# skygazer42/realtime-video-analytics-32streams

Measured on AMD Instinct MI355X. Metric: aggregate detected FPS across streams + p99 per-frame latency, 32x1080p30, higher is better.
Workload: dtype f16

## Files before the change

### include/rva.h

```cpp
#ifndef RVA_H
#define RVA_H

#include <stdint.h>

#ifdef __cplusplus
extern "C" {
#endif

#define RVA_ABI_VERSION 1

enum rva_status {
    RVA_OK = 0,
    RVA_ERR_ARG = 1,
    RVA_ERR_HIP = 2,
    RVA_ERR_CAPACITY = 3,
    RVA_ERR_UNAVAILABLE = 4
};

enum rva_dtype { RVA_F16 = 0, RVA_F32 = 1, RVA_F64 = 2  };

typedef struct rva_ctx rva_ctx;
typedef struct rva_tracker rva_tracker;
typedef void *rva_stream_t;

// ... 104 lines not shown
#define RVA_SNAPSHOT_SLOTS 8
int rva_tracker_snapshot_async(rva_tracker *trk, int slot, rva_stream_t stream);
int rva_tracker_snapshot_fetch(rva_tracker *trk, int slot, int wait, int64_t *ids, int32_t *cls, int32_t *age,
                               int32_t *hits, double *conf, double *boxes, int32_t *last_det,
                               int32_t *counts);

int rva_tracker_snapshot_status(rva_tracker *trk, int slot, int32_t *emitted, int32_t *processed, int32_t *flags);

int rva_tracker_state(rva_tracker *trk, int64_t *next_id, int *flags, rva_stream_t stream);
int rva_tracker_set_next_id(rva_tracker *trk, int64_t next_id, rva_stream_t stream);

int rva_conv_cout_pad(int Cout);
int rva_conv_num_variants(void);
const char *rva_conv_variant_name(int variant);
int rva_conv2d_nhwc_f16(rva_ctx *ctx, const void *in, int ldi, const void *weights, const float *bias,
                        void *out, int ldo, const void *residual, int ldr, int batch, int H, int W, int Cin,
                        int Cout, int ksize, int stride, int act, rva_stream_t stream);
int rva_conv2d_nhwc_f16_v(rva_ctx *ctx, const void *in, int ldi, const void *weights, const float *bias,
                          void *out, int ldo, const void *residual, int ldr, int batch, int H, int W, int Cin,
                          int Cout, int ksize, int stride, int act, int variant, rva_stream_t stream);
int rva_conv2d_nhwc_f16_rows(rva_ctx *ctx, const void *in, int ldi, const void *weights, const float *bias,
                             void *out, int ldo, const void *residual, int ldr, int batch, int H, int W, int Cin,
                             int Cout, int ksize, int stride, int act, int variant, int y0, int y1, rva_stream_t stream);
int rva_conv_rows_through(int k, int stride, int H_in, int lo, int hi, int32_t *out_lo, int32_t *out_hi);
int rva_conv1x1_upcat_f16(rva_ctx *ctx, const void *low, int ld_low, int c_low, const void *skip, int ld_skip,
                          int c_skip, const void *weights, const float *bias, void *out, int ldo, int batch,
                          int H, int W, int Cout, int act, int variant, rva_stream_t stream);
int rva_conv1x1_head_f16(rva_ctx *ctx, const void *in, int ldi, const void *weights, const float *bias, int batch,
                         int H, int W, int Cin, int Cout, int mode, void *out, int nc, int anchors_total,
                         int anchor_offset, float stride_px, int variant, rva_stream_t stream);
int rva_conv1x1_head_box32_f16(rva_ctx *ctx, const void *in, int ldi, const void *weights, const float *bias, int batch,
                               int H, int W, int Cin, void *out, float *boxes32, int nc, int anchors_total, int anchor_offset,
                               float stride_px, int variant, rva_stream_t stream);
int rva_stem_conv_f16(rva_ctx *ctx, const void *in_planar, const void *weights, const float *bias,
                      void *out, int ldo, int batch, int H, int W, int Cout, rva_stream_t stream);

int rva_c2f_pair32_f16(rva_ctx *ctx, const void *in, int ldi, const void *w1, const float *b1, const void *w2, const float *b2, void *out,
                       int ldo, int batch, int H, int W, rva_stream_t stream);

int rva_stem2_f16(rva_ctx *ctx, const void *in_planar, const void *w1, const float *b1, const void *w2, const float *b2,
                  void *out, int ldo, int batch, int H, int W, rva_stream_t stream);
int rva_stem2_f16_rows(rva_ctx *ctx, const void *in_planar, const void *w1, const float *b1, const void *w2, const float *b2,
                       void *out, int ldo, int batch, int H, int W, int y0, int y1, rva_stream_t stream);

int rva_sppf_pool3_nhwc_f16(rva_ctx *ctx, const void *in, int ldi, void *out1, void *out2, void *out3, int ldo,
                            int batch, int H, int W, int C, rva_stream_t stream);
int rva_maxpool5_nhwc_f16(rva_ctx *ctx, const void *in, int ldi, void *out, int ldo, int batch, int H,
                          int W, int C, rva_stream_t stream);
int rva_upsample2x_nhwc_f16(rva_ctx *ctx, const void *in, int ldi, void *out, int ldo, int batch, int H,
                            int W, int C, rva_stream_t stream);
int rva_yolo_head_f16(rva_ctx *ctx, const void *box_logits, int ldb, const void *cls_logits, int ldc,
                      void *out, int batch, int h, int w, int nc, int anchors_total, int anchor_offset,
                      float stride, rva_stream_t stream);
int rva_yolo_head3_f16(rva_ctx *ctx, const void *const *box_logits, const int32_t *ldb, const void *const *cls_logits,
                       const int32_t *ldc, void *out, int batch, const int32_t *h, const int32_t *w, int nc,
                       int anchors_total, const float *strides, rva_stream_t stream);
int rva_yolo_head_box32_f16(rva_ctx *ctx, const void *box_logits, int ldb, const void *cls_logits, int ldc, void *out,
                            float *boxes32, int batch, int h, int w, int nc, int anchors_total, int anchor_offset, float stride,
                            rva_stream_t stream);
int rva_yolo_head3_box32_f16(rva_ctx *ctx, const void *const *box_logits, const int32_t *ldb, const void *const *cls_logits,
                             const int32_t *ldc, void *out, float *boxes32, int batch, const int32_t *h, const int32_t *w, int nc,
                             int anchors_total, const float *strides, rva_stream_t stream);

int rva_conv_f32_num_variants(void);
int rva_conv2d_nhwc_f32_v(rva_ctx *ctx, const void *in, int ldi, const void *weights, const float *bias,
                          void *out, int ldo, const void *residual, int ldr, int batch, int H, int W, int Cin,
                          int Cout, int ksize, int stride, int act, int variant, rva_stream_t stream);
int rva_stem_conv_f32(rva_ctx *ctx, const void *in_planar, const void *weights, const float *bias,
                      void *out, int ldo, int batch, int H, int W, int Cout, rva_stream_t stream);
int rva_maxpool5_nhwc_f32(rva_ctx *ctx, const void *in, int ldi, void *out, int ldo, int batch, int H,
                          int W, int C, rva_stream_t stream);
int rva_upsample2x_nhwc_f32(rva_ctx *ctx, const void *in, int ldi, void *out, int ldo, int batch, int H,
                            int W, int C, rva_stream_t stream);
int rva_yolo_head_f32(rva_ctx *ctx, const void *box_logits, int ldb, const void *cls_logits, int ldc,
                      void *out, int batch, int h, int w, int nc, int anchors_total, int anchor_offset,
                      float stride, rva_stream_t stream);

#define RVA_PLAN_NO_STEM2 1
#define RVA_PLAN_NO_CIN_PAD 2
#define RVA_PLAN_NO_PAIR32 4
#define RVA_PLAN_F32 8
#define RVA_PLAN_BOX_F32 16
typedef struct rva_yolov8_plan rva_yolov8_plan;
typedef struct rva_yolov8_desc {
    int32_t batch, height, width;
    int32_t widths[5];
    int32_t depth_backbone[4];
    int32_t depth_head;
    int32_t nc, reg_max;
    int32_t n_convs;
    int32_t flags;
} rva_yolov8_desc;
typedef struct rva_conv_weights {
    const float *weight;
    const float *bias;
    int32_t cout, cin, k, stride;
} rva_conv_weights;
int rva_yolov8_plan_create(rva_ctx *ctx, const rva_yolov8_desc *desc, const rva_conv_weights *convs, rva_yolov8_plan **out);
void rva_yolov8_plan_destroy(rva_yolov8_plan *plan);
int rva_yolov8_plan_info(const rva_yolov8_plan *plan, int32_t *anchors, int32_t *out_rows, int32_t *n_steps, int32_t *n_tunable,
                         int32_t *quiet_step);
int rva_yolov8_plan_output_layout(const rva_yolov8_plan *plan, int64_t *total_bytes, int64_t *boxes_offset);
int rva_yolov8_plan_run(rva_yolov8_plan *plan, const void *input, void *output, rva_stream_t stream);
int rva_yolov8_plan_run_lanes(rva_yolov8_plan *plan, const void *input, void *output, rva_stream_t stream, rva_stream_t side1,
                              rva_stream_t side2);
int rva_yolov8_plan_run_range(rva_yolov8_plan *plan, const void *input, void *output, int first, int last, rva_stream_t stream);
int rva_yolov8_plan_tunable_desc(const rva_yolov8_plan *plan, int index, char *buf, int len);
int rva_yolov8_plan_launch_tunable(rva_yolov8_plan *plan, int index, int variant, void *output, rva_stream_t stream);
int rva_yolov8_plan_set_variant(rva_yolov8_plan *plan, int index, int variant);
int rva_yolov8_plan_get_variant(const rva_yolov8_plan *plan, int index);
int rva_yolov8_plan_set_static_rows(rva_yolov8_plan *plan, int top, int bottom);
int rva_yolov8_plan_run_n(rva_yolov8_plan *plan, const void *input, void *output, int n, rva_stream_t stream);
int rva_yolov8_plan_run_lanes_n(rva_yolov8_plan *plan, const void *input, void *output, int n, rva_stream_t stream, rva_stream_t side1,
                                rva_stream_t side2);
int rva_yolov8_plan_run_range_n(rva_yolov8_plan *plan, const void *input, void *output, int n, int first, int last, rva_stream_t stream);
// ... 179 lines not shown
```

### realtime_video_analytics_32streams_amd/_native.py

```python
from __future__ import annotations

import ctypes as C
import os
import shutil
import subprocess
from pathlib import Path
from typing import Optional

PKG = Path(__file__).resolve().parent
ROOT = PKG.parent
CSRC = PKG / "csrc"
LIB_PATH = Path(os.environ["RVA_LIB_PATH"]) if os.environ.get("RVA_LIB_PATH") else PKG / "librva.so"
SOURCES = ["rva_ctx.hip", "rva_preprocess.hip", "rva_postprocess.hip", "rva_tracker.hip", "rva_conv.hip", "rva_conv_f32.hip", "rva_plan.hip", "rva_clip.hip",
           "rva_clip3d.hip", "rva_clip3d_f16.hip", "rva_clip_f16.hip", "rva_resnet.hip", "rva_resnet_f16.hip", "rva_gates.hip", "rva_decode.hip", "rva_preview.hip", "rva_jpeg.hip"]
HIPCC_FLAGS = ["--offload-arch=gfx950", "-O3", "-fPIC", "-shared", "-std=c++17", "-ffp-contract=off",
               "-Wall", "-Wno-unused-function"]

RVA_OK, RVA_ERR_ARG, RVA_ERR_HIP, RVA_ERR_CAPACITY, RVA_ERR_UNAVAILABLE = range(5)
RVA_F16, RVA_F32, RVA_F64 = 0, 1, 2
NORM_IMAGENET_F32, NORM_VIDEO_F32, NORM_IMAGENET_F64 = 0, 1, 2
LAYOUT_NCHW, LAYOUT_CNHW = 0, 1
RVA_MAX_BATCH = 64
RVA_CODEC_H264, RVA_CODEC_HEVC = 0, 1

# ... 26 lines not shown
class CnnLstmWeights(C.Structure):
    NAMES = ("conv1_w", "conv1_b", "conv2_w", "conv2_b", "w_ih1", "b1", "w_hh1", "w_ih2", "w_hh2", "b2", "head_w", "head_b")
    _fields_ = [(n, C.POINTER(C.c_float)) for n in NAMES]


class Cnn3dDesc(C.Structure):
    _fields_ = [("height", C.c_int32), ("width", C.c_int32), ("frames", C.c_int32), ("classes", C.c_int32), ("max_clips", C.c_int32)]


class Cnn3dWeights(C.Structure):
    NAMES = ("conv1_w", "conv1_b", "conv2_w", "conv2_b", "conv3_w", "conv3_b", "head_w", "head_b")
    _fields_ = [(n, C.POINTER(C.c_float)) for n in NAMES]


class ResNetDesc(C.Structure):
    _fields_ = [("height", C.c_int32), ("width", C.c_int32), ("classes", C.c_int32), ("top_k", C.c_int32), ("max_frames", C.c_int32)]


class ResNetWeights(C.Structure):
    NAMES = ("stem_w", "stem_b") + tuple(f"c{i}_{x}" for i in range(19) for x in "wb") + ("head_w", "head_b")
    _fields_ = [(n, C.POINTER(C.c_float)) for n in NAMES]


class PreviewItem(C.Structure):
    _fields_ = [("y", C.c_void_p), ("uv", C.c_void_p), ("out_bgr", C.c_void_p)] + [
        (n, C.c_int32) for n in ("pitch", "src_w", "src_h", "ratio", "dst_w", "dst_h", "rect_first", "n_rects", "glyph_first", "n_glyphs")]


RVA_PLAN_NO_STEM2 = 1
RVA_PLAN_NO_CIN_PAD = 2
RVA_PLAN_NO_PAIR32 = 4
RVA_PLAN_F32 = 8
RVA_PLAN_BOX_F32 = 16


def _stale() -> bool:
    if not LIB_PATH.exists():
        return True
    t = LIB_PATH.stat().st_mtime
    deps = [CSRC / s for s in SOURCES] + [CSRC / "rva_internal.h", CSRC / "rva_mfma_f32.h", CSRC / "rva_mfma_f16.h", ROOT / "include" / "rva.h"]
    return any(d.exists() and d.stat().st_mtime > t for d in deps)


def build(force: bool = False, verbose: bool = False) -> Path:
    if not force and not _stale():
        return LIB_PATH
    hipcc = shutil.which("hipcc") or "/opt/rocm/bin/hipcc"
    if not Path(hipcc).exists():
        if LIB_PATH.exists():
            return LIB_PATH
        raise RuntimeError("hipcc not found and librva.so is not built")
    cmd = [hipcc, *HIPCC_FLAGS, f"-I{ROOT / 'include'}", "-o", str(LIB_PATH), *[str(CSRC / s) for s in SOURCES], "-ldl"]
    if verbose:
        print(" ".join(cmd))
    subprocess.check_call(cmd, cwd=str(CSRC))
    return LIB_PATH


_LIB: Optional[C.CDLL] = None
_P = C.c_void_p


def lib() -> C.CDLL:
    global _LIB
    if _LIB is not None:
        return _LIB
# ... 45 lines not shown
        "rva_tracker_set_gates": (C.c_int, [_P, i32p, i32p, i32p, i32p, C.c_int]),
        "rva_tracker_snapshot_status": (C.c_int, [_P, C.c_int, _P, _P, C.POINTER(C.c_int32)]),
        "rva_tracker_new_counts": (_P, [_P]),
        "rva_tracker_assign_ids": (C.c_int, [_P, _P, C.c_int, i32p, _P]),
        "rva_tracker_read": (C.c_int, [_P, C.c_int, C.c_int, _P, _P, _P, _P, _P, _P, _P, i32p, _P]),
        "rva_tracker_read_all": (C.c_int, [_P, _P, _P, _P, _P, _P, _P, _P, _P, _P]),
        "rva_tracker_snapshot_async": (C.c_int, [_P, C.c_int, _P]),
        "rva_tracker_snapshot_fetch": (C.c_int, [_P, C.c_int, C.c_int, _P, _P, _P, _P, _P, _P, _P, _P]),
        "rva_tracker_state": (C.c_int, [_P, i64p, C.POINTER(C.c_int), _P]),
        "rva_tracker_set_next_id": (C.c_int, [_P, C.c_int64, _P]),
        "rva_preview_nv12": (C.c_int, [_P, _P, _P, C.c_int, C.c_int, C.c_int, C.c_int, _P, C.c_int, C.c_int, _P, _P, C.c_int, _P, C.c_int,
                                       C.c_int, _P]),
        "rva_decode_available": (C.c_int, [C.c_char_p, C.c_int]),
        "rva_decoder_create": (C.c_int, [_P, C.c_int, C.c_int, C.POINTER(_P)]),
        "rva_decoder_destroy": (None, [_P]),
        "rva_decoder_feed": (C.c_int, [_P, C.c_char_p, C.c_int, C.c_int64, C.c_int]),
        "rva_decoder_next_frame": (C.c_int, [_P, C.POINTER(_P), C.POINTER(_P), i32p, i32p, i32p, i64p, i32p]),
        "rva_decoder_release": (C.c_int, [_P, C.c_int]),
        "rva_motion_nv12_batch": (C.c_int, [_P, pp, pp, i32p, pp, pp, C.c_int, C.c_int, C.c_int, _P, _P]),
        "rva_motion_nv12_masked_batch": (C.c_int, [_P, pp, pp, i32p, pp, pp, pp, C.c_int, C.c_int, C.c_int, _P, _P]),
        "rva_motion_bgr_batch": (C.c_int, [_P, pp, i32p, pp, pp, C.c_int, C.c_int, C.c_int, _P, _P]),
        "rva_preprocess_nv12_masked_batch": (C.c_int, [_P, pp, pp, i32p, pp, C.c_int, C.c_int, C.c_int, _P, C.c_int, C.c_int,
                                                       C.c_int, C.POINTER(Letterbox), _P]),
        "rva_resize_nv12_to_bgr_batch": (C.c_int, [_P, pp, pp, i32p, pp, C.c_int, C.c_int, C.c_int, _P, C.c_int, C.c_int, _P]),
        "rva_tracker_set_box_scale": (C.c_int, [_P, f64p]),
        "rva_conv_cout_pad": (C.c_int, [C.c_int]),
        "rva_conv_num_variants": (C.c_int, []),
        "rva_conv_variant_name": (C.c_char_p, [C.c_int]),
        "rva_conv2d_nhwc_f16": (C.c_int, [_P, _P, C.c_int, _P, _P, _P, C.c_int, _P, C.c_int] + [C.c_int] * 8 + [_P]),
        "rva_conv2d_nhwc_f16_v": (C.c_int, [_P, _P, C.c_int, _P, _P, _P, C.c_int, _P, C.c_int] + [C.c_int] * 9 + [_P]),
        "rva_conv2d_nhwc_f16_rows": (C.c_int, [_P, _P, C.c_int, _P, _P, _P, C.c_int, _P, C.c_int] + [C.c_int] * 11 + [_P]),
        "rva_conv_rows_through": (C.c_int, [C.c_int] * 5 + [i32p, i32p]),
        "rva_stem2_f16_rows": (C.c_int, [_P, _P, _P, _P, _P, _P, _P, C.c_int, C.c_int, C.c_int, C.c_int, C.c_int, C.c_int, _P]),
        "rva_stem_conv_f16": (C.c_int, [_P, _P, _P, _P, _P, C.c_int, C.c_int, C.c_int, C.c_int, C.c_int, _P]),
        "rva_stem2_f16": (C.c_int, [_P, _P, _P, _P, _P, _P, _P, C.c_int, C.c_int, C.c_int, C.c_int, _P]),
        "rva_c2f_pair32_f16": (C.c_int, [_P, _P, C.c_int, _P, _P, _P, _P, _P, C.c_int, C.c_int, C.c_int, C.c_int, _P]),
        "rva_conv1x1_head_f16": (C.c_int, [_P, _P, C.c_int, _P, _P, C.c_int, C.c_int, C.c_int, C.c_int, C.c_int, C.c_int, _P, C.c_int,
                                           C.c_int, C.c_int, C.c_float, C.c_int, _P]),
        "rva_conv1x1_head_box32_f16": (C.c_int, [_P, _P, C.c_int, _P, _P, C.c_int, C.c_int, C.c_int, C.c_int, _P, _P, C.c_int,
                                                 C.c_int, C.c_int, C.c_float, C.c_int, _P]),
        "rva_yolo_head_box32_f16": (C.c_int, [_P, _P, C.c_int, _P, C.c_int, _P, _P, C.c_int, C.c_int, C.c_int, C.c_int, C.c_int,
                                              C.c_int, C.c_float, _P]),
        "rva_yolo_head3_box32_f16": (C.c_int, [_P, pp, i32p, pp, i32p, _P, _P, C.c_int, i32p, i32p, C.c_int, C.c_int,
                                               C.POINTER(C.c_float), _P]),
        "rva_conv1x1_upcat_f16": (C.c_int, [_P, _P, C.c_int, C.c_int, _P, C.c_int, C.c_int, _P, _P, _P, C.c_int, C.c_int, C.c_int,
                                            C.c_int, C.c_int, C.c_int, C.c_int, _P]),
        "rva_yolo_head3_f16": (C.c_int, [_P, pp, i32p, pp, i32p, _P, C.c_int, i32p, i32p, C.c_int, C.c_int, C.POINTER(C.c_float), _P]),
        "rva_sppf_pool3_nhwc_f16": (C.c_int, [_P, _P, C.c_int, _P, _P, _P, C.c_int, C.c_int, C.c_int, C.c_int, C.c_int, _P]),
        "rva_maxpool5_nhwc_f16": (C.c_int, [_P, _P, C.c_int, _P, C.c_int, C.c_int, C.c_int, C.c_int, C.c_int, _P]),
        "rva_upsample2x_nhwc_f16": (C.c_int, [_P, _P, C.c_int, _P, C.c_int, C.c_int, C.c_int, C.c_int, C.c_int, _P]),
        "rva_yolo_head_f16": (C.c_int, [_P, _P, C.c_int, _P, C.c_int, _P, C.c_int, C.c_int, C.c_int, C.c_int, C.c_int,
                                        C.c_int, C.c_float, _P]),
        "rva_conv_f32_num_variants": (C.c_int, []),
        "rva_conv2d_nhwc_f32_v": (C.c_int, [_P, _P, C.c_int, _P, _P, _P, C.c_int, _P, C.c_int] + [C.c_int] * 9 + [_P]),
        "rva_stem_conv_f32": (C.c_int, [_P, _P, _P, _P, _P, C.c_int, C.c_int, C.c_int, C.c_int, C.c_int, _P]),
        "rva_maxpool5_nhwc_f32": (C.c_int, [_P, _P, C.c_int, _P, C.c_int, C.c_int, C.c_int, C.c_int, C.c_int, _P]),
        "rva_upsample2x_nhwc_f32": (C.c_int, [_P, _P, C.c_int, _P, C.c_int, C.c_int, C.c_int, C.c_int, C.c_int, _P]),
        "rva_yolo_head_f32": (C.c_int, [_P, _P, C.c_int, _P, C.c_int, _P, C.c_int, C.c_int, C.c_int, C.c_int, C.c_int,
                                        C.c_int, C.c_float, _P]),
        "rva_yolov8_plan_create": (C.c_int, [_P, C.POINTER(YoloV8Desc), C.POINTER(ConvWeights), C.POINTER(_P)]),
        "rva_yolov8_plan_destroy": (None, [_P]),
        "rva_yolov8_plan_info": (C.c_int, [_P, i32p, i32p, i32p, i32p, i32p]),
        "rva_yolov8_plan_output_layout": (C.c_int, [_P, i64p, i64p]),
        "rva_yolov8_plan_run": (C.c_int, [_P, _P, _P, _P]),
        "rva_yolov8_plan_run_lanes": (C.c_int, [_P, _P, _P, _P, _P, _P]),
        "rva_yolov8_plan_run_range": (C.c_int, [_P, _P, _P, C.c_int, C.c_int, _P]),
# ... 59 lines not shown
        raise RuntimeError("librva.so ABI version mismatch; rebuild it")
    _LIB = L
    return L


EXPORTS = [
    "rva_abi_version", "rva_create", "rva_destroy", "rva_last_error", "rva_reserve", "rva_letterbox_meta",
    "rva_preprocess_nv12_batch", "rva_preprocess_nv12_content_batch", "rva_preprocess_bgr_batch", "rva_preprocess_clip_nv12_batch",
    "rva_preprocess_clip_bgr_batch", "rva_profile_next_preprocess", "rva_preprocess_frames_nv12_batch", "rva_preprocess_frames_bgr_batch", "rva_postprocess_batch", "rva_post_status", "rva_post_filter_stats", "rva_tracker_create",
    "rva_tracker_destroy", "rva_tracker_update_f32", "rva_tracker_update_f64", "rva_tracker_update_gated_f32",
    "rva_tracker_set_gates", "rva_tracker_snapshot_status", "rva_tracker_new_counts",
    "rva_tracker_assign_ids", "rva_tracker_read", "rva_tracker_read_all", "rva_tracker_snapshot_async",
    "rva_tracker_snapshot_fetch", "rva_tracker_state",
    "rva_tracker_set_next_id", "rva_preview_nv12", "rva_decode_available", "rva_decoder_create", "rva_decoder_destroy", "rva_decoder_feed",
    "rva_decoder_next_frame", "rva_decoder_release", "rva_motion_nv12_batch", "rva_motion_nv12_masked_batch", "rva_motion_bgr_batch",
    "rva_preprocess_nv12_masked_batch", "rva_resize_nv12_to_bgr_batch", "rva_tracker_set_box_scale", "rva_conv_cout_pad", "rva_conv_num_variants", "rva_conv_variant_name", "rva_conv2d_nhwc_f16", "rva_conv2d_nhwc_f16_v", "rva_stem_conv_f16", "rva_stem2_f16", "rva_c2f_pair32_f16",
    "rva_conv1x1_head_f16", "rva_conv1x1_upcat_f16", "rva_sppf_pool3_nhwc_f16", "rva_maxpool5_nhwc_f16", "rva_upsample2x_nhwc_f16", "rva_yolo_head_f16", "rva_yolo_head3_f16",
    "rva_conv_f32_num_variants", "rva_conv2d_nhwc_f32_v", "rva_stem_conv_f32", "rva_maxpool5_nhwc_f32", "rva_upsample2x_nhwc_f32",
    "rva_yolo_head_f32",
    "rva_postprocess_boxes_batch", "rva_conv1x1_head_box32_f16", "rva_yolo_head_box32_f16", "rva_yolo_head3_box32_f16",
    "rva_yolov8_plan_output_layout",
    "rva_yolov8_plan_create", "rva_yolov8_plan_destroy", "rva_yolov8_plan_info", "rva_yolov8_plan_run", "rva_yolov8_plan_run_lanes",
    "rva_yolov8_plan_run_range", "rva_yolov8_plan_tunable_desc", "rva_yolov8_plan_launch_tunable", "rva_yolov8_plan_set_variant",
    "rva_yolov8_plan_get_variant", "rva_yolov8_plan_set_static_rows", "rva_yolov8_plan_step_rows", "rva_yolov8_plan_run_n",
    "rva_yolov8_plan_run_lanes_n", "rva_yolov8_plan_run_range_n", "rva_yolov8_plan_primed_images", "rva_conv2d_nhwc_f16_rows",
    "rva_stem2_f16_rows", "rva_conv_rows_through", "rva_cnnlstm_plan_create", "rva_cnnlstm_plan_destroy", "rva_cnnlstm_plan_info", "rva_cnnlstm_plan_run",
    "rva_cnnlstm_plan_run_post", "rva_cnnlstm_plan_stage", "rva_cnnlstm_f16_plan_create", "rva_cnnlstm_f16_plan_destroy", "rva_cnnlstm_f16_plan_info",
    "rva_cnnlstm_f16_plan_run", "rva_cnnlstm_f16_plan_run_post", "rva_cnnlstm_f16_plan_stage", "rva_cnn3d_plan_create", "rva_cnn3d_plan_destroy", "rva_cnn3d_plan_info", "rva_cnn3d_plan_run",
    "rva_cnn3d_plan_run_post", "rva_cnn3d_plan_stage", "rva_cnn3d_f16_plan_create", "rva_cnn3d_f16_plan_destroy", "rva_cnn3d_f16_plan_info",
    "rva_cnn3d_f16_plan_run", "rva_cnn3d_f16_plan_run_post", "rva_cnn3d_f16_plan_stage", "rva_resnet_plan_create", "rva_resnet_plan_destroy", "rva_resnet_plan_info",
    "rva_resnet_plan_run", "rva_resnet_plan_run_post", "rva_resnet_plan_stage", "rva_resnet_f16_plan_create", "rva_resnet_f16_plan_destroy",
    "rva_resnet_f16_plan_info", "rva_resnet_f16_plan_run", "rva_resnet_f16_plan_run_post", "rva_resnet_f16_plan_stage", "rva_jpeg_max_bytes", "rva_jpeg_encode_bgr", "rva_jpeg_status",
    "rva_jpeg_batch_create", "rva_jpeg_batch_destroy", "rva_jpeg_batch_encode", "rva_preview_nv12_batch",
]


class Context:

    def __init__(self, device: int = 0):
        L = lib()
        h = _P()
        rc = L.rva_create(device, C.byref(h))
        if rc != RVA_OK or not h:
            raise RuntimeError(
                f"rva_create(device={device}) failed with status {rc}: no usable HIP device. "
                "The MI355X hot path has no CPU fallback.")
        self.handle = h
        self.device = device

    def check(self, rc: int, what: str = "") -> None:
        if rc != RVA_OK:
            msg = lib().rva_last_error(self.handle)
            raise RuntimeError(f"{what or 'librva'} failed (status {rc}): {msg.decode() if msg else ''}")

    def close(self) -> None:
        if getattr(self, "handle", None):
            lib().rva_destroy(self.handle)
            self.handle = None

    def __del__(self):
        try:
            self.close()
        except Exception:
            pass


# ... 17 lines not shown
```

### realtime_video_analytics_32streams_amd/csrc/rva_conv.hip

```cpp
#include <hip/hip_fp16.h>

#include <cstdlib>

#include "rva_internal.h"

namespace {

typedef _Float16 h8 __attribute__((ext_vector_type(8)));
typedef float f4 __attribute__((ext_vector_type(4)));
typedef unsigned int u4 __attribute__((ext_vector_type(4)));

struct ConvArgs {
    const __half *in; int ldi;
    const __half *w;
    const float *bias;
    __half *out; int ldo;
    union {
        const __half *res;
        float *hbox;
    };
    int ldr;
    int CoutPad;
    __half *hout; int hmode, hnc, hA, ha0, hW, hHW; float hstride;
    const __half *in2; int ldi2, c_split;
// ... 996 lines not shown
        for (int t = 0; t < 16; ++t) mx = fmaxf(mx, v[t]);
        float se = 0.f, sw = 0.f;
#pragma unroll
        for (int t = 0; t < 16; ++t) { const float e = __expf(v[t] - mx); se += e; sw += e * (float)t; }
        d[s] = sw / se;
    }
    const float ax = (float)(i % a.w) + 0.5f, ay = (float)(i / a.w) + 0.5f;
    const float x1 = ax - d[0], y1 = ay - d[1], x2 = ax + d[2], y2 = ay + d[3];
    __half *o = a.out + (size_t)b * (4 + a.nc) * a.A + a.a0 + i;
    o[0] = __float2half_rn((x1 + x2) * 0.5f * a.stride);
    o[(size_t)a.A] = __float2half_rn((y1 + y2) * 0.5f * a.stride);
    o[(size_t)2 * a.A] = __float2half_rn((x2 - x1) * a.stride);
    o[(size_t)3 * a.A] = __float2half_rn((y2 - y1) * a.stride);
    if constexpr (BOX32) {
        float *o32 = box32 + (size_t)b * 4 * a.A + a.a0 + i;
        o32[0] = (x1 + x2) * 0.5f * a.stride;
        o32[(size_t)a.A] = (y1 + y2) * 0.5f * a.stride;
        o32[(size_t)2 * a.A] = (x2 - x1) * a.stride;
        o32[(size_t)3 * a.A] = (y2 - y1) * a.stride;
    }
    const __half *cp = a.cls + pix * a.ldc;
    for (int c = 0; c < a.nc; c += 8) {
        const uint4 q = *reinterpret_cast<const uint4 *>(cp + c);
        const __half2 *hq = reinterpret_cast<const __half2 *>(&q);
#pragma unroll
        for (int t = 0; t < 4; ++t) {
            const float2 f = __half22float2(hq[t]);
            o[(size_t)(4 + c + 2 * t) * a.A] = __float2half_rn(__builtin_amdgcn_rcpf(1.0f + __expf(-f.x)));
            o[(size_t)(5 + c + 2 * t) * a.A] = __float2half_rn(__builtin_amdgcn_rcpf(1.0f + __expf(-f.y)));
        }
    }
}

struct BigArgs {
    const __half *in; int ldi;
    const __half *w; const float *bias;
    __half *out; int ldo;
    const __half *res; int ldr;
    int H, W, Cin, Cout, CoutPad, act, n_tiles, M, m_tiles;
};

typedef __attribute__((address_space(3))) void *lds_vptr;
typedef const __attribute__((address_space(1))) void *glb_vptr;

template <int N> __device__ __forceinline__ void wait_vm() { asm volatile("s_waitcnt vmcnt(%0)" ::"n"(N) : "memory"); }

__device__ __forceinline__ void lds_dma16(unsigned voff, const void *sbase, unsigned m0v)
{
    const unsigned long long b = (unsigned long long)(size_t)sbase;
    const unsigned lo = __builtin_amdgcn_readfirstlane((unsigned)b), hi = __builtin_amdgcn_readfirstlane((unsigned)(b >> 32));
    const unsigned long long sb = ((unsigned long long)hi << 32) | lo;
    const unsigned m0s = __builtin_amdgcn_readfirstlane(m0v);
    asm volatile("s_mov_b32 m0, %2\n\ts_nop 0\n\tglobal_load_lds_dwordx4 %0, %1" ::"v"(voff), "s"(sb), "s"(m0s) : "memory");
}
__device__ __forceinline__ void lds_dma16_masked(unsigned voff, const void *sbase, unsigned m0v, unsigned long long mask)
{
    const unsigned long long b = (unsigned long long)(size_t)sbase;
    const unsigned lo = __builtin_amdgcn_readfirstlane((unsigned)b), hi = __builtin_amdgcn_readfirstlane((unsigned)(b >> 32));
    const unsigned long long sb = ((unsigned long long)hi << 32) | lo;
    const unsigned m0s = __builtin_amdgcn_readfirstlane(m0v);
    const unsigned mlo = __builtin_amdgcn_readfirstlane((unsigned)mask), mhi = __builtin_amdgcn_readfirstlane((unsigned)(mask >> 32));
    const unsigned long long ms = ((unsigned long long)mhi << 32) | mlo;
    asm volatile("s_mov_b32 m0, %2\n\ts_mov_b64 exec, %3\n\tglobal_load_lds_dwordx4 %0, %1\n\ts_mov_b64 exec, -1" ::"v"(voff), "s"(sb), "s"(m0s), "s"(ms) : "memory");
}
__device__ __forceinline__ unsigned lds_addr(const void *p) { return (unsigned)(size_t)(lds_vptr)p; }
__device__ __forceinline__ void wait_vm_n(int n)
{
    switch (n) {
    case 0: wait_vm<0>(); break;
    case 1: wait_vm<1>(); break;
    case 2: wait_vm<2>(); break;
    case 3: wait_vm<3>(); break;
    case 4: wait_vm<4>(); break;
    case 5: wait_vm<5>(); break;
    case 6: wait_vm<6>(); break;
    case 7: wait_vm<7>(); break;
    case 8: wait_vm<8>(); break;
    case 9: wait_vm<9>(); break;
    case 10: wait_vm<10>(); break;
    case 11: wait_vm<11>(); break;
    case 12: wait_vm<12>(); break;
    default: wait_vm<12>(); break;
    }
}

template <int BM, int BN, int WGM, int WGN, int NSLOT>
__global__ void __launch_bounds__(512) __attribute__((amdgpu_waves_per_eu(NSLOT == 2 ? 4 : 2))) k_conv3_big(BigArgs a)
{
    static_assert(WGM * WGN == 8, "eight waves");
    static_assert(NSLOT == 2 || NSLOT == 3, "ring depth");
    constexpr int TM = BM / WGM, TN = BN / WGN, FM = TM / 16, FN = TN / 16;
    constexpr int APIECES = (BM + 2 + 15) / 16;
    constexpr int WPIECES = 3 * BN / 16;
    constexpr int PIECES = APIECES + WPIECES;
    constexpr int SLOTH = PIECES * 512;
    constexpr int NP = (PIECES + 7) / 8;
    extern __shared__ __attribute__((aligned(16))) unsigned char smem[];
    __half *ring = (__half *)smem;

    const int tid = threadIdx.x, lane = tid & 63;
    const int wv = __builtin_amdgcn_readfirstlane(tid >> 6);
    const int wm = wv % WGM, wn = wv / WGM;
    const int n_tile = (blockIdx.x >> 3) % a.n_tiles, m_tile = ((blockIdx.x >> 3) / a.n_tiles) * 8 + (blockIdx.x & 7);
    if (m_tile >= a.m_tiles) return;
    const int P0 = m_tile * BM, n0 = n_tile * BN;
    const int HW = a.H * a.W;
    const int cpt = a.Cin >> 5;
    const int nsteps = 3 * cpt;
    const int wrow = 9 * a.Cin;

    const int lrow = lane >> 2, lp = lane & 3;
    const int my_pieces = (PIECES - wv + 7) / 8;
    unsigned poff0[NP], poff1[NP], poff2[NP];
#pragma unroll
    for (int k = 0; k < NP; ++k) {
        const int idx = wv + 8 * k;
        if (idx < APIECES) {
            const int r = idx * 16 + lrow;
            const unsigned c = (unsigned)(((lp - 2 * (r >> 2)) & 3) * 16);
            const int q1 = P0 - 1 + r;
// ... 129 lines not shown
                    if (!((vm[j] >> (vsh + dx)) & 1)) bf[0][j] = hz;
                }
#pragma unroll
                for (int i = 0; i < FN; ++i) {
                    const h8 a1 = *reinterpret_cast<const h8 *>(wb + swz32(dx * BN + wn * TN + i * 16 + (lane & 15), ch));
#pragma unroll
                    for (int j = 0; j < FM; ++j) acc[i][j] = __builtin_amdgcn_mfma_f32_16x16x32_f16(a1, bf[0][j], acc[i][j], 0, 0, 0);
                }
            }
        }
        if (NSLOT == 3 && more && !early) BIG_ISSUE();
        STAMP(5);
    }
    __syncthreads();

    constexpr int SROW = BN + 8;
    __half *stage = (__half *)smem;
#pragma unroll
    for (int i = 0; i < FN; ++i) {
        const int co = wn * TN + 16 * i + (lane >> 4) * 4;
        const float4 bv = bvs[i];
#pragma unroll
        for (int j = 0; j < FM; ++j) {
            float v0 = acc[i][j][0] + bv.x, v1 = acc[i][j][1] + bv.y, v2 = acc[i][j][2] + bv.z, v3 = acc[i][j][3] + bv.w;
            if (a.act) { v0 = silu_f(v0); v1 = silu_f(v1); v2 = silu_f(v2); v3 = silu_f(v3); }
            const int px = wm * TM + 16 * j + (lane & 15);
            __half2 lo = __floats2half2_rn(v0, v1), hi = __floats2half2_rn(v2, v3);
            uint2 pk;
            pk.x = *reinterpret_cast<uint32_t *>(&lo);
            pk.y = *reinterpret_cast<uint32_t *>(&hi);
            *reinterpret_cast<uint2 *>(stage + (size_t)px * SROW + co) = pk;
        }
    }
    __syncthreads();
    constexpr int CPR = BN / 8;
#pragma unroll 4
    for (int q = tid; q < BM * CPR; q += 512) {
        const int row = q / CPR, pc = q - row * CPR;
        const int co = n0 + pc * 8;
        const int m = P0 + row;
        if (m < a.M && co < a.Cout) {
            uint4 v = *reinterpret_cast<const uint4 *>(stage + (size_t)row * SROW + pc * 8);
            if (a.res) {
                const uint4 r = *reinterpret_cast<const uint4 *>(a.res + (size_t)m * a.ldr + co);
                __half2 *vh = reinterpret_cast<__half2 *>(&v);
                const __half2 *rh = reinterpret_cast<const __half2 *>(&r);
#pragma unroll
                for (int u = 0; u < 4; ++u) {
                    const float2 x = __half22float2(vh[u]), y = __half22float2(rh[u]);
                    vh[u] = __floats2half2_rn(x.x + y.x, x.y + y.y);
                }
            }
            *reinterpret_cast<uint4 *>(a.out + (size_t)m * a.ldo + co) = v;
        }
    }
    STAMP(6);
}

#undef BIG_ISSUE
#undef BIG_ISSUE_ADVANCE
#undef BIG_ISSUE_PIECE

template <int BM, int BN, int WGM, int WGN, int NSLOT>
hipError_t launch_big(BigArgs &a, hipStream_t s)
{
    constexpr size_t ring = (size_t)NSLOT * ((BM + 2 + 15) / 16 + 3 * BN / 16) * 1024;
    constexpr size_t st = (size_t)BM * (BN + 8) * 2;
    constexpr size_t smem = ring > st ? ring : st;
    static_assert(smem <= 160 * 1024, "LDS budget");
    if (a.Cin % 32 || a.CoutPad % 4 || a.M >= (1 << 24)) return hipErrorInvalidValue;
    if ((size_t)a.M * a.ldi * 2 >= (1ull << 32) || (size_t)a.CoutPad * 9 * a.Cin * 2 >= (1ull << 32)) return hipErrorInvalidValue;
    if (hipError_t e = rva_func_smem((const void *)k_conv3_big<BM, BN, WGM, WGN, NSLOT>, smem); e != hipSuccess) return e;
    a.n_tiles = rva_ceil_div(a.Cout, BN);
    a.m_tiles = rva_ceil_div(a.M, BM);
    k_conv3_big<BM, BN, WGM, WGN, NSLOT><<<rva_ceil_div(a.m_tiles, 8) * 8 * a.n_tiles, 512, smem, s>>>(a);
    return hipGetLastError();
}

struct RunArgs {
    const __half *in; int ldi;
    const __half *w; const float *bias;
    __half *out; int ldo;
    const __half *res; int ldr;
    int H, W, Cin, Cout, CoutPad, act, n_tiles, M, m_tiles, apieces, map_off;
};

template <int BM, int BN, int WGM, int WGN, bool NOSEL = false, bool PADO = false>
__global__ void __launch_bounds__(512) __attribute__((amdgpu_waves_per_eu(BN <= 64 && BM <= 320 ? 4 : 2))) k_conv3_run(RunArgs a)
{
    static_assert(WGM * WGN == 8, "eight waves");
    constexpr int TM = BM / WGM, TN = BN / WGN, FM = TM / 16, FN = TN / 16;
    constexpr int WPIECES = 3 * BN / 16;
    constexpr int NPW = (WPIECES + 7) / 8;
    constexpr int MAXA = 5;
    extern __shared__ __attribute__((aligned(16))) unsigned char smem[];
    const int tid = threadIdx.x, lane = tid & 63;
    const int wv = __builtin_amdgcn_readfirstlane(tid >> 6);
    const int wm = wv % WGM, wn = wv / WGM;
    const int n_tile = (blockIdx.x >> 3) % a.n_tiles, m_tile = ((blockIdx.x >> 3) / a.n_tiles) * 8 + (blockIdx.x & 7);
    if (m_tile >= a.m_tiles) return;
    const int P0 = m_tile * BM, n0 = n_tile * BN;
    const int HW = a.H * a.W;
    const int cpt = a.Cin >> 5;
    const int nsteps = 3 * cpt;
    const int wrow = 9 * a.Cin;
    const int apieces = a.apieces;
    __half *act0 = (__half *)smem;
    __half *wt0 = act0 + (size_t)2 * apieces * 512;
    const unsigned lds_act = lds_addr(act0), lds_w = lds_addr(wt0);

    const int lrow = lane >> 2, lp = lane & 3;
    unsigned aoff[MAXA], woff[NPW];
    const int Wp = PADO ? a.W + 1 : a.W, HWp = (a.H + 1) * Wp;
    const float inv_wp = 1.0f / (float)Wp, inv_hwp = 1.0f / (float)HWp;
    unsigned long long amask[PADO ? MAXA : 1];
    auto pixel_of = [&](int pos) {
        if (pos < 0) return -1;
        const int b = div_s(pos, HWp, inv_hwp), rem = pos - b * HWp, yy = div_s(rem, Wp, inv_wp), xx = rem - yy * Wp;
        const int m = (b * a.H + yy) * a.W + xx;
        return (yy < a.H && xx < a.W && m < a.M) ? m : -1;
    };
// ... 123 lines not shown
        RUN_LOAD(0, 0);
        RUN_LOAD(1, 1);
        RUN_MFMA(0, 0);
        if (!early) RUN_ISSUE();
        RUN_LOAD(0, 2);
        RUN_MFMA(1, 1);
        RUN_MFMA(0, 2);
#undef RUN_LOAD
#undef RUN_MFMA
#undef RUN_ISSUE
        cc = ncc; dy = ndy;
        STAMP(5);
    }
    __syncthreads();

    constexpr int SROW = BN + 8;
    __half *stage = (__half *)smem;
#pragma unroll
    for (int i = 0; i < FN; ++i) {
        const int co = wn * TN + 16 * i + (lane >> 4) * 4;
        const float4 bv = bvs[i];
#pragma unroll
        for (int j = 0; j < FM; ++j) {
            float v0 = acc[i][j][0] + bv.x, v1 = acc[i][j][1] + bv.y, v2 = acc[i][j][2] + bv.z, v3 = acc[i][j][3] + bv.w;
            if (a.act) { v0 = silu_f(v0); v1 = silu_f(v1); v2 = silu_f(v2); v3 = silu_f(v3); }
            const int px = wm * TM + 16 * j + (lane & 15);
            __half2 lo = __floats2half2_rn(v0, v1), hi = __floats2half2_rn(v2, v3);
            uint2 pk;
            pk.x = *reinterpret_cast<uint32_t *>(&lo);
            pk.y = *reinterpret_cast<uint32_t *>(&hi);
            *reinterpret_cast<uint2 *>(stage + (size_t)px * SROW + co) = pk;
        }
    }
    __syncthreads();
    constexpr int CPR = BN / 8;
#pragma unroll 4
    for (int q = tid; q < BM * CPR; q += 512) {
        const int row = q / CPR, pc = q - row * CPR;
        const int co = n0 + pc * 8;
        const int m = PADO ? rowmap[row] : P0 + row;
        if ((PADO ? m >= 0 : m < a.M) && co < a.Cout) {
            uint4 v = *reinterpret_cast<const uint4 *>(stage + (size_t)row * SROW + pc * 8);
            if (a.res) {
                const uint4 r = *reinterpret_cast<const uint4 *>(a.res + (size_t)m * a.ldr + co);
                __half2 *vh = reinterpret_cast<__half2 *>(&v);
                const __half2 *rh = reinterpret_cast<const __half2 *>(&r);
#pragma unroll
                for (int u = 0; u < 4; ++u) {
                    const float2 x = __half22float2(vh[u]), y = __half22float2(rh[u]);
                    vh[u] = __floats2half2_rn(x.x + y.x, x.y + y.y);
                }
            }
            *reinterpret_cast<uint4 *>(a.out + (size_t)m * a.ldo + co) = v;
        }
    }
    STAMP(6);
}

template <int BM, int BN, int WGM, int WGN, bool NOSEL = false, bool PADO = false>
hipError_t launch_run(RunArgs &a, hipStream_t s)
{
    if (a.Cin % 32 || a.CoutPad % 4 || a.W > 160 || a.M >= (1 << 24)) return hipErrorInvalidValue;
    if ((size_t)a.M * a.ldi * 2 >= (1ull << 32) || (size_t)a.CoutPad * 9 * a.Cin * 2 >= (1ull << 32)) return hipErrorInvalidValue;
    const int wp = PADO ? a.W + 1 : a.W;
    a.apieces = rva_ceil_div(BM + 2 * wp + 2, 16);
    if (a.apieces > 8 * 5) return hipErrorInvalidValue;
    const size_t ring = (size_t)(2 * a.apieces + 2 * (3 * BN / 16)) * 1024;
    const size_t st = (size_t)BM * (BN + 8) * 2;
    size_t smem = ring > st ? ring : st;
    long mp = a.M;
    if (PADO) {
        const int batch = a.M / (a.H * a.W);
        mp = (long)batch * (a.H + 1) * (a.W + 1);
        if (a.M % (a.H * a.W) || mp >= (1l << 24)) return hipErrorInvalidValue;
        a.map_off = (int)smem;
        smem += (size_t)BM * 4;
    }
    if (smem > 160 * 1024) return hipErrorInvalidValue;
    if (hipError_t e = rva_func_smem((const void *)k_conv3_run<BM, BN, WGM, WGN, NOSEL, PADO>, 160 * 1024); e != hipSuccess) return e;
    a.n_tiles = rva_ceil_div(a.Cout, BN);
    a.m_tiles = (int)((mp + BM - 1) / BM);
    k_conv3_run<BM, BN, WGM, WGN, NOSEL, PADO><<<rva_ceil_div(a.m_tiles, 8) * 8 * a.n_tiles, 512, smem, s>>>(a);
    return hipGetLastError();
}

template <int BM, int BN, int WGM, int WGN>
__global__ void __launch_bounds__(512) __attribute__((amdgpu_waves_per_eu(BM <= 128 && BN <= 64 ? 4 : 2))) k_conv3_s2run(RunArgs a)
{
    static_assert(WGM * WGN == 8, "eight waves");
    constexpr int TM = BM / WGM, TN = BN / WGN, FM = TM / 16, FN = TN / 16;
    constexpr int WPIECES = 3 * BN / 16, NPW = (WPIECES + 7) / 8;
    constexpr int BMO = (BM + 1 + 15) / 16 * 16;
    constexpr int AP = (BMO + BM) / 16, MAXA = (AP + 7) / 8;
    extern __shared__ __attribute__((aligned(16))) unsigned char smem[];
    const int tid = threadIdx.x, lane = tid & 63;
    const int wv = __builtin_amdgcn_readfirstlane(tid >> 6);
    const int wm = wv % WGM, wn = wv / WGM;
    const int n_tile = (blockIdx.x >> 3) % a.n_tiles, m_tile = ((blockIdx.x >> 3) / a.n_tiles) * 8 + (blockIdx.x & 7);
    if (m_tile >= a.m_tiles) return;
    const int P0 = m_tile * BM, n0 = n_tile * BN;
    const int Ho = a.H >> 1, Wo = a.W >> 1, Wp = Wo + 1, HWp = Ho * Wp;
    const int cpt = a.Cin >> 5, nsteps = 3 * cpt, wrow = 9 * a.Cin;
    __half *act0 = (__half *)smem;
    __half *wt0 = act0 + (size_t)3 * AP * 512;
    const unsigned lds_act = lds_addr(act0), lds_w = lds_addr(wt0);
    const int lrow = lane >> 2, lp = lane & 3;
    const float inv_wp = 1.0f / (float)Wp, inv_hwp = 1.0f / (float)HWp;
    const int batch = a.M / (Ho * Wo);
    unsigned aoff[MAXA], woff[NPW];
    unsigned long long am1[MAXA], am0[MAXA];
#pragma unroll
    for (int k = 0; k < MAXA; ++k) {
        const int r = (wv + 8 * k) * 16 + lrow;
        const bool odd = r < BMO;
        const int pos = odd ? P0 - 1 + r : P0 + (r - BMO);
// ... 125 lines not shown
                    const float2 x = __half22float2(vh[u]), y = __half22float2(rh[u]);
                    vh[u] = __floats2half2_rn(x.x + y.x, x.y + y.y);
                }
            }
            *reinterpret_cast<uint4 *>(a.out + (size_t)m * a.ldo + co) = v;
        }
    }
}

template <int BM, int BN, int WGM, int WGN>
hipError_t launch_s2run(RunArgs &a, hipStream_t s)
{
    constexpr int BMO = (BM + 1 + 15) / 16 * 16, AP = (BMO + BM) / 16;
    if (a.Cin % 32 || a.CoutPad % 4 || (a.H & 1) || (a.W & 1)) return hipErrorInvalidValue;
    const int Ho = a.H / 2, Wo = a.W / 2;
    if (Ho <= 0 || Wo <= 0 || a.M % (Ho * Wo)) return hipErrorInvalidValue;
    const long batch = a.M / (Ho * Wo);
    const long mp = batch * Ho * (Wo + 1);
    if (mp >= (1l << 24)) return hipErrorInvalidValue;
    if ((size_t)batch * a.H * a.W * a.ldi * 2 >= (1ull << 32) || (size_t)a.CoutPad * 9 * a.Cin * 2 >= (1ull << 32)) return hipErrorInvalidValue;
    const size_t ring = (size_t)(3 * AP + 2 * (3 * BN / 16)) * 1024;
    const size_t st = (size_t)BM * (BN + 8) * 2;
    size_t smem = ring > st ? ring : st;
    a.map_off = (int)smem;
    smem += (size_t)BM * 4;
    if (smem > 160 * 1024) return hipErrorInvalidValue;
    if (hipError_t e = rva_func_smem((const void *)k_conv3_s2run<BM, BN, WGM, WGN>, 160 * 1024); e != hipSuccess) return e;
    a.n_tiles = rva_ceil_div(a.Cout, BN);
    a.m_tiles = (int)((mp + BM - 1) / BM);
    k_conv3_s2run<BM, BN, WGM, WGN><<<rva_ceil_div(a.m_tiles, 8) * 8 * a.n_tiles, 512, smem, s>>>(a);
    return hipGetLastError();
}

template <int BM, int BN, int WGM, int WGN>
__global__ void __launch_bounds__(512) __attribute__((amdgpu_waves_per_eu(2))) k_conv3_chunk(RunArgs a)
{
    static_assert(WGM * WGN == 8, "eight waves");
    constexpr int TM = BM / WGM, TN = BN / WGN, FM = TM / 16, FN = TN / 16;
    static_assert(TM % 16 == 0 && TN % 16 == 0, "whole fragments per wave");
    constexpr int WPIECES = 9 * BN / 16;
    constexpr int NPW = (WPIECES + 7) / 8;
    constexpr int MAXA = 5;
    extern __shared__ __attribute__((aligned(16))) unsigned char smem[];
    const int tid = threadIdx.x, lane = tid & 63;
    const int wv = __builtin_amdgcn_readfirstlane(tid >> 6);
    const int wm = wv % WGM, wn = wv / WGM;
    const int n_tile = (blockIdx.x >> 3) % a.n_tiles, m_tile = ((blockIdx.x >> 3) / a.n_tiles) * 8 + (blockIdx.x & 7);
    if (m_tile >= a.m_tiles) return;
    const int P0 = m_tile * BM, n0 = n_tile * BN;
    const int HW = a.H * a.W;
    const int cpt = a.Cin >> 5;
    const int wrow = 9 * a.Cin;
    const int apieces = a.apieces;
    __half *act0 = (__half *)smem;
    __half *wt0 = act0 + (size_t)2 * apieces * 512;
    const unsigned lds_act = lds_addr(act0), lds_w = lds_addr(wt0);

    const int lrow = lane >> 2, lp = lane & 3;
    unsigned aoff[MAXA], woff[NPW];
#pragma unroll
    for (int k = 0; k < MAXA; ++k) {
        const int r = (wv + 8 * k) * 16 + lrow;
        const int q = min(max(P0 - a.W - 1 + r, 0), a.M - 1);
        aoff[k] = (unsigned)q * (unsigned)(a.ldi * 2) + (unsigned)(((lp - 2 * (r >> 2)) & 3) * 16);
    }
#pragma unroll
    for (int k = 0; k < NPW; ++k) {
        const int rw = (wv + 8 * k) * 16 + lrow;
// ... 73 lines not shown
        if (!early && cc + 1 < cpt) CHUNK_ISSUE(cc + 1);
        CHUNK_LOAD(0, 2); CHUNK_MFMA(1, 1);
        CHUNK_LOAD(1, 3); CHUNK_MFMA(0, 2);
        CHUNK_LOAD(0, 4); CHUNK_MFMA(1, 3);
        CHUNK_LOAD(1, 5); CHUNK_MFMA(0, 4);
        CHUNK_LOAD(0, 6); CHUNK_MFMA(1, 5);
        CHUNK_LOAD(1, 7); CHUNK_MFMA(0, 6);
        CHUNK_LOAD(0, 8); CHUNK_MFMA(1, 7);
        CHUNK_MFMA(0, 8);
#undef CHUNK_LOAD
#undef CHUNK_MFMA
    }
#undef CHUNK_ISSUE
    __syncthreads();

    constexpr int SROW = BN + 8;
    __half *stage = (__half *)smem;
#pragma unroll
    for (int i = 0; i < FN; ++i) {
        const int co = wn * TN + 16 * i + (lane >> 4) * 4;
        const float4 bv = bvs[i];
#pragma unroll
        for (int j = 0; j < FM; ++j) {
            float v0 = acc[i][j][0] + bv.x, v1 = acc[i][j][1] + bv.y, v2 = acc[i][j][2] + bv.z, v3 = acc[i][j][3] + bv.w;
            if (a.act) { v0 = silu_f(v0); v1 = silu_f(v1); v2 = silu_f(v2); v3 = silu_f(v3); }
            const int px = wm * TM + 16 * j + (lane & 15);
            __half2 lo = __floats2half2_rn(v0, v1), hi = __floats2half2_rn(v2, v3);
            uint2 pk;
            pk.x = *reinterpret_cast<uint32_t *>(&lo);
            pk.y = *reinterpret_cast<uint32_t *>(&hi);
            *reinterpret_cast<uint2 *>(stage + (size_t)px * SROW + co) = pk;
        }
    }
    __syncthreads();
    constexpr int CPR = BN / 8;
#pragma unroll 4
    for (int q = tid; q < BM * CPR; q += 512) {
        const int row = q / CPR, pc = q - row * CPR;
        const int co = n0 + pc * 8;
        const int m = P0 + row;
        if (m < a.M && co < a.Cout) {
            uint4 v = *reinterpret_cast<const uint4 *>(stage + (size_t)row * SROW + pc * 8);
            if (a.res) {
                const uint4 r = *reinterpret_cast<const uint4 *>(a.res + (size_t)m * a.ldr + co);
                __half2 *vh = reinterpret_cast<__half2 *>(&v);
                const __half2 *rh = reinterpret_cast<const __half2 *>(&r);
#pragma unroll
                for (int u = 0; u < 4; ++u) {
                    const float2 x = __half22float2(vh[u]), y = __half22float2(rh[u]);
                    vh[u] = __floats2half2_rn(x.x + y.x, x.y + y.y);
                }
            }
            *reinterpret_cast<uint4 *>(a.out + (size_t)m * a.ldo + co) = v;
        }
    }
}

template <int BM, int BN, int WGM, int WGN>
hipError_t launch_chunk(RunArgs &a, hipStream_t s)
{
    if (a.Cin % 32 || a.CoutPad % 4 || a.W > 160 || a.M >= (1 << 24)) return hipErrorInvalidValue;
    if ((size_t)a.M * a.ldi * 2 >= (1ull << 32) || (size_t)a.CoutPad * 9 * a.Cin * 2 >= (1ull << 32)) return hipErrorInvalidValue;
    a.apieces = rva_ceil_div(BM + 2 * a.W + 2, 16);
    if (a.apieces > 8 * 5) return hipErrorInvalidValue;
    const size_t ring = (size_t)(2 * a.apieces + 2 * (9 * BN / 16)) * 1024;
    const size_t st = (size_t)BM * (BN + 8) * 2;
    const size_t smem = ring > st ? ring : st;
    if (smem > 160 * 1024) return hipErrorInvalidValue;
    if (hipError_t e = rva_func_smem((const void *)k_conv3_chunk<BM, BN, WGM, WGN>, 160 * 1024); e != hipSuccess) return e;
    a.n_tiles = rva_ceil_div(a.Cout, BN);
    a.m_tiles = rva_ceil_div(a.M, BM);
    k_conv3_chunk<BM, BN, WGM, WGN><<<rva_ceil_div(a.m_tiles, 8) * 8 * a.n_tiles, 512, smem, s>>>(a);
    return hipGetLastError();
}

template <int BM, int BN, int WGM, int WGN, int NSLOT, int KS, int BK, bool UP = false, bool HEAD = false, int SUB = 1>
__global__ void __launch_bounds__(512)
    __attribute__((amdgpu_waves_per_eu(NSLOT * SUB * (BM + BN) * BK * 2 <= 80 * 1024 ? 4 : 2))) k_conv_gbig(ConvArgs a)
{
    static_assert(WGM * WGN == 8, "eight waves");
    static_assert(BK == 32 || BK == 64, "K-step of 32 or 64 channels");
    static_assert(SUB == 1 || NSLOT == 2, "several K-steps per barrier: two-slot ring");
    static_assert(!UP || (KS == 1 && BK == 64), "the upsample + concat source form exists for 1x1 convolutions");
    constexpr int TM = BM / WGM, TN = BN / WGN, FM = TM / 16, FN = TN / 16;
    constexpr int RPP = 512 / BK;
    constexpr int LPR = BK / 8;
    constexpr int APIECES = BM / RPP, WPIECES = BN / RPP;
    constexpr int NA = (APIECES + 7) / 8, NW = (WPIECES + 7) / 8;
    constexpr int SLOTH = (BM + BN) * BK;
    constexpr int TAPS = KS * KS, PAD = KS / 2;
    extern __shared__ __attribute__((aligned(16))) unsigned char smem[];
    __half *ring = (__half *)smem;

    const int tid = threadIdx.x, lane = tid & 63;
    const int wv = __builtin_amdgcn_readfirstlane(tid >> 6);
    const int wm = wv % WGM, wn = wv / WGM;
    const int n_tile = (blockIdx.x >> 3) % a.n_tiles, m_tile = ((blockIdx.x >> 3) / a.n_tiles) * 8 + (blockIdx.x & 7);
    if (m_tile >= a.m_tiles) return;
    const int P0 = m_tile * BM, n0 = n_tile * BN;
    const int HoWo = a.wrows * a.Wo;
    const int cpt = a.Cin / BK;
    const int nsteps = TAPS * cpt;
    const int wrow = TAPS * a.Cin;

    const int lrow = lane / LPR, lp = lane % LPR;
// ... 132 lines not shown
            for (int i = 0; i < FN; ++i) {
                const int r = wr + 16 * i;
                const h8 af = *reinterpret_cast<const h8 *>(wb + (BK == 64 ? r * 64 + ((ks * 4 + (lane >> 4)) ^ xr) * 8 : swz32(r, lane >> 4)));
#pragma unroll
                for (int j = 0; j < FM; ++j) acc[i][j] = __builtin_amdgcn_mfma_f32_16x16x32_f16(af, bf[j], acc[i][j], 0, 0, 0);
            }
        }
      }
        if (more && !early) GB_ISSUE();
    }
#undef GB_ISSUE
    __syncthreads();

    constexpr int SROW = BN + 8;
    __half *stage = (__half *)smem;
#pragma unroll
    for (int i = 0; i < FN; ++i) {
        const int co = wn * TN + 16 * i + (lane >> 4) * 4;
        const float4 bv = bvs[i];
#pragma unroll
        for (int j = 0; j < FM; ++j) {
            float v0 = acc[i][j][0] + bv.x, v1 = acc[i][j][1] + bv.y, v2 = acc[i][j][2] + bv.z, v3 = acc[i][j][3] + bv.w;
            if (a.act) { v0 = silu_f(v0); v1 = silu_f(v1); v2 = silu_f(v2); v3 = silu_f(v3); }
            const int px = wm * TM + 16 * j + (lane & 15);
            __half2 lo = __floats2half2_rn(v0, v1), hi = __floats2half2_rn(v2, v3);
            uint2 pk;
            pk.x = *reinterpret_cast<uint32_t *>(&lo);
            pk.y = *reinterpret_cast<uint32_t *>(&hi);
            *reinterpret_cast<uint2 *>(stage + (size_t)px * SROW + co) = pk;
        }
    }
    __syncthreads();
    if constexpr (HEAD) {
        for (int r = tid; r < BM; r += 512) {
            const int m = P0 + r;
            if (m >= a.M) continue;
            const int b = m / a.hHW, i = m - b * a.hHW;
            __half *o = a.hout + (size_t)b * (4 + a.hnc) * a.hA + a.ha0 + i;
            const __half *row = stage + (size_t)r * SROW;
            if (a.hmode == 1) {
                float d[4];
#pragma unroll
                for (int sd = 0; sd < 4; ++sd) {
                    float v[16], mx = -1e30f;
                    const uint4 q0 = *reinterpret_cast<const uint4 *>(row + sd * 16), q1 = *reinterpret_cast<const uint4 *>(row + sd * 16 + 8);
                    const __half2 *h0 = reinterpret_cast<const __half2 *>(&q0), *h1 = reinterpret_cast<const __half2 *>(&q1);
#pragma unroll
                    for (int t = 0; t < 4; ++t) {
                        float2 f = __half22float2(h0[t]); v[2 * t] = f.x; v[2 * t + 1] = f.y;
                        f = __half22float2(h1[t]); v[8 + 2 * t] = f.x; v[9 + 2 * t] = f.y;
                    }
#pragma unroll
                    for (int t = 0; t < 16; ++t) mx = fmaxf(mx, v[t]);
                    float se = 0.f, sw = 0.f;
#pragma unroll
                    for (int t = 0; t < 16; ++t) { const float e = __expf(v[t] - mx); se += e; sw += e * (float)t; }
                    d[sd] = sw / se;
                }
                const float ax = (float)(i % a.hW) + 0.5f, ay = (float)(i / a.hW) + 0.5f;
                const float x1 = ax - d[0], y1 = ay - d[1], x2 = ax + d[2], y2 = ay + d[3];
                o[0] = __float2half_rn((x1 + x2) * 0.5f * a.hstride);
                o[(size_t)a.hA] = __float2half_rn((y1 + y2) * 0.5f * a.hstride);
                o[(size_t)2 * a.hA] = __float2half_rn((x2 - x1) * a.hstride);
                o[(size_t)3 * a.hA] = __float2half_rn((y2 - y1) * a.hstride);
                if (a.hbox) {
                    float *o32 = a.hbox + (size_t)b * 4 * a.hA + a.ha0 + i;
                    o32[0] = (x1 + x2) * 0.5f * a.hstride;
                    o32[(size_t)a.hA] = (y1 + y2) * 0.5f * a.hstride;
                    o32[(size_t)2 * a.hA] = (x2 - x1) * a.hstride;
                    o32[(size_t)3 * a.hA] = (y2 - y1) * a.hstride;
                }
            } else {
                const int cend = min(BN, a.Cout - n0);
                for (int c = 0; c < cend; c += 8) {
                    const uint4 q = *reinterpret_cast<const uint4 *>(row + c);
                    const __half2 *hq = reinterpret_cast<const __half2 *>(&q);
#pragma unroll
                    for (int t = 0; t < 4; ++t) {
                        const float2 f = __half22float2(hq[t]);
                        o[(size_t)(4 + n0 + c + 2 * t) * a.hA] = __float2half_rn(__builtin_amdgcn_rcpf(1.0f + __expf(-f.x)));
                        o[(size_t)(5 + n0 + c + 2 * t) * a.hA] = __float2half_rn(__builtin_amdgcn_rcpf(1.0f + __expf(-f.y)));
                    }
                }
            }
        }
        return;
    }
    constexpr int CPR = BN / 8;
    const int wskip = (a.Ho - a.wrows) * a.Wo;
#pragma unroll 4
    for (int q = tid; q < BM * CPR; q += 512) {
        const int row = q / CPR, pc = q - row * CPR;
        const int co = n0 + pc * 8;
        const int mw = P0 + row;
        if (mw < a.M && co < a.Cout) {
            const int m = wskip ? mw + div_s(mw, HoWo, inv_howo) * wskip + a.wy0 * a.Wo : mw;
            uint4 v = *reinterpret_cast<const uint4 *>(stage + (size_t)row * SROW + pc * 8);
            if (a.res) {
                const uint4 r = *reinterpret_cast<const uint4 *>(a.res + (size_t)m * a.ldr + co);
                __half2 *vh = reinterpret_cast<__half2 *>(&v);
                const __half2 *rh = reinterpret_cast<const __half2 *>(&r);
#pragma unroll
                for (int u = 0; u < 4; ++u) {
                    const float2 x = __half22float2(vh[u]), y = __half22float2(rh[u]);
                    vh[u] = __floats2half2_rn(x.x + y.x, x.y + y.y);
                }
            }
            *reinterpret_cast<uint4 *>(a.out + (size_t)m * a.ldo + co) = v;
        }
    }
}

template <int BM, int BN, int WGM, int WGN, int NSLOT, int KS, int BK, bool UP = false, bool HEAD = false, int SUB = 1>
hipError_t launch_gbig1(ConvArgs &a, hipStream_t s)
{
    constexpr size_t ring = (size_t)NSLOT * SUB * (BM + BN) * BK * 2;
// ... 928 lines not shown
    g.B = c.batch; g.Ho = c.a.Ho; g.Wo = c.a.Wo; g.CoutPad = c.cpad; g.y0 = c.y0; g.y1 = c.y1;
    return launch_patch<STRIDE, CIN, CO, NWV, NBUF, RPW>(g, c.num_cus, c.s);
}

template <int CIN, int CO, int SW, int RPW>
hipError_t v_patch2(const ConvCall &c)
{
    if (!is_3x3(c, 1) || c.a.Cin != CIN || c.a.Cout > CO) return hipErrorInvalidValue;
    S2Args g = family_args<S2Args>(c);
    g.B = c.batch; g.Ho = c.a.Ho; g.Wo = c.a.Wo; g.CoutPad = c.cpad; g.y0 = c.y0; g.y1 = c.y1;
    return launch_patch2<CIN, CO, SW, RPW>(g, c.num_cus, c.s);
}

template <hipError_t (*LAUNCH)(RunArgs &, hipStream_t), int STRIDE = 1>
hipError_t v_run(const ConvCall &c)
{
    if (c.windowed()) return hipErrorInvalidValue;
    if (!is_3x3(c, STRIDE)) return hipErrorInvalidValue;
    RunArgs g = dma3_args<RunArgs>(c);
    return LAUNCH(g, c.s);
}

#ifdef RVA_EXPERIMENTS
template <int BM, int BN, int WGM, int WGN>
hipError_t v_run_nosel(const ConvCall &c)
{
    const char *nosel = getenv("RVA_NOSEL");
    if (!is_3x3(c, 1) || !nosel || nosel[0] != '1') return hipErrorInvalidValue;
    RunArgs g = dma3_args<RunArgs>(c);
    return launch_run<BM, BN, WGM, WGN, true>(g, c.s) == hipSuccess ? hipSuccess : hipErrorInvalidValue;
}
#endif

hipError_t launch_variant(int variant, const ConvCall &c);

inline bool auto_picks_gather(int Cin, int ksize, int stride) { return Cin % 64 == 0 && ((ksize == 3 && stride == 2) || (ksize == 1 && stride == 1)); }

inline bool first_choice_fits(const ConvCall &c, int pick)
{
    const ConvArgs &a = c.a;
    if (pick == 37) {
        const long m = (long)c.sel_batch * (c.y1 - c.y0) * a.Wo;
        return m < (1 << 24) && (size_t)a.H * a.W * (size_t)(c.sel_batch + 1) * a.ldi * 2 < (1ull << 32);
    }
    const long m = (long)c.sel_batch * a.Ho * a.Wo;
    return m < (1 << 24) && (size_t)m * a.ldi * 2 < (1ull << 32);
}

hipError_t v_auto(const ConvCall &c)
{
    const ConvArgs &a = c.a;
    const int cpad = c.cpad;
    const bool bn128 = cpad % 128 == 0;
    const long selM = (long)c.sel_batch * a.Ho * a.Wo;
    int pick = 0;
    if (is_3x3(c, 1) && a.Cin % 32 == 0)
        pick = bn128 ? (selM * a.Cout >= 20000000L ? 25 : 21) : (selM >= 100000 ? 31 : 23);
    else if (auto_picks_gather(a.Cin, c.ksize, a.stride))
        pick = 37;
    if (pick && !first_choice_fits(c, pick)) pick = 0;
    if (c.windowed()) return pick == 37 ? launch_variant(37, c) : hipErrorInvalidValue;
    if (pick) {
        if (launch_variant(pick, c) == hipSuccess) return hipSuccess;
        (void)hipGetLastError();
    }
    if (a.stride == 1) {
// ... 5 lines not shown
            if (e == hipErrorInvalidValue && t256 * (cpad / 64) >= want) e = launch_variant(5, c);
            if (e == hipErrorInvalidValue && bn128 && t128 * (cpad / 128) >= want) e = launch_variant(8, c);
            if (e == hipErrorInvalidValue) e = launch_variant(6, c);
        } else if (a.CinPad % 128 == 0) {
            const long t256 = (selM + 255) / 256;
            if (bn128 && t256 * (cpad / 128) >= want) e = launch_variant(7, c);
            if (e == hipErrorInvalidValue && t256 * (cpad / 64) >= want) e = launch_variant(5, c);
            if (e == hipErrorInvalidValue) e = launch_variant(6, c);
        } else {
            const long t256 = (selM + 255) / 256;
            e = launch_variant(t256 * (cpad / 64) >= want ? 5 : 6, c);
        }
        if (e != hipErrorInvalidValue) return e;
        (void)hipGetLastError();
    }
    const bool small = (selM + 255) / 256 * (cpad / (bn128 ? 128 : 64)) < 512;
    return launch_variant(bn128 ? (small ? 4 : 3) : (small ? 2 : 1), c);
}

#define RVA_GATHER64_TILES(X)                                                                       \
    X(33, "gb<256,128>", 256, 128, 4, 2, 3)                            \
    X(34, "gb<128,128>", 128, 128, 2, 4, 3)                                               \
    X(35, "gb<256,64>", 256, 64, 4, 2, 3)                                                \
    X(36, "gb<128,64>", 128, 64, 2, 4, 3)                              \
    X(37, "gb2<128,128>", 128, 128, 2, 4, 2)                           \
    X(38, "gb2<256,64>", 256, 64, 4, 2, 2)                             \
    X(39, "gb2<192,128>", 192, 128, 4, 2, 2)

struct ConvVariant {
    int number;
    const char *name;
    hipError_t (*launch)(const ConvCall &);
    bool rows = false;
};

constexpr ConvVariant kConvVariants[] = {
    {0, "auto", v_auto},
    {1, "gather<64,64>", v_gather<64, 64>},
    {2, "gather<64,32>", v_gather<64, 32>},
    {3, "gather<128,64>", v_gather<128, 64>},
    {4, "gather<128,32>", v_gather<128, 32>},
    {5, "res<64,64>", v_res<64, 64>},
    {6, "res<64,32>", v_res<64, 32>},
    {7, "res<128,64>", v_res<128, 64>},
    {8, "res<128,32>", v_res<128, 32>},
    {9, "row<64,64>", v_row<64, 64>},
    {10, "row<64,32>", v_row<64, 32>},
    {11, "row<128,64>", v_row<128, 64>},
    {12, "row<128,32>", v_row<128, 32>},
    {13, "g64<64,64>", v_gather<64, 64, 64>},
    {14, "g64<64,32>", v_gather<64, 32, 64>},
    {15, "g64<128,64>", v_gather<128, 64, 64>},
    {16, "g64<128,32>", v_gather<128, 32, 64>},
    {17, "row2<64,64>", v_row<64, 64, true>},
    {18, "row2<64,32>", v_row<64, 32, true>},
    {19, "row2<128,64>", v_row<128, 64, true>},
    {20, "row2<128,32>", v_row<128, 32, true>},
    {21, "big<256,128>", v_big<256, 128, 4, 2, 3>},
    {22, "big<128,128>", v_big<128, 128, 2, 4, 3>},
    {23, "big<256,64>", v_big<256, 64, 4, 2, 3>},
    {24, "big<128,64>", v_big<128, 64, 2, 4, 3>},
    {25, "big2<192,128>", v_big<192, 128, 4, 2, 2>},
    {26, "big2<128,128>", v_big<128, 128, 2, 4, 2>},
    {27, "big2<256,64>", v_big<256, 64, 4, 2, 2>},
    {28, "big2<128,64>", v_big<128, 64, 2, 4, 2>},
    {29, "big2<224,128>", v_big<224, 128, 2, 4, 2>},
    {30, "big2<160,128>", v_big<160, 128, 2, 4, 2>},
    {31, "big2<384,64>", v_big<384, 64, 8, 1, 2>},
    {32, "big2<320,64>", v_big<320, 64, 4, 2, 2>},
#define RVA_ROW(n, name, ...) {n, name, v_gbig<__VA_ARGS__>, true},
    RVA_GATHER64_TILES(RVA_ROW)
#undef RVA_ROW
    {40, "gb32<256,64>", v_gbig<256, 64, 4, 2, 3, 32>, true},
    {41, "gb32<128,64>", v_gbig<128, 64, 2, 4, 3, 32>, true},
    {42, "gb32_2<256,64>", v_gbig<256, 64, 4, 2, 2, 32>, true},
    {43, "s2patch", v_patch<2, 32, 64, 4, 1>, true},
    {44, "s1patch4", v_patch<1, 32, 32, 4, 1>, true},
    {45, "s1patch8", v_patch<1, 32, 32, 8, 1>, true},
    {46, "p64x4db", v_patch<1, 64, 64, 4, 2>, true},
    {47, "p64x8", v_patch<1, 64, 64, 8, 1>, true},
    {48, "p64x4", v_patch<1, 64, 64, 4, 1>, true},
    {49, "p64x8db", v_patch<1, 64, 64, 8, 2>, true},
    {50, "p64x4r2db", v_patch<1, 64, 64, 4, 2, 2>, true},
    {51, "p64x8r2", v_patch<1, 64, 64, 8, 1, 2>, true},
    {52, "run<256,64>", v_run<launch_run<256, 64, 4, 2>>},
    {53, "run<128,64>", v_run<launch_run<128, 64, 2, 4>>},
    {54, "run<384,64>", v_run<launch_run<384, 64, 8, 1>>},
    {55, "run<192,128>", v_run<launch_run<192, 128, 4, 2>>},
    {56, "run<256,128>", v_run<launch_run<256, 128, 4, 2>>},
    {57, "run<128,128>", v_run<launch_run<128, 128, 2, 4>>},
    {58, "run<224,128>", v_run<launch_run<224, 128, 2, 4>>},
    {59, "run<160,128>", v_run<launch_run<160, 128, 2, 4>>},
    {60, "run<320,64>", v_run<launch_run<320, 64, 4, 2>>},
    {61, "p64h32x8", v_patch<1, 64, 32, 8, 1, 1>, true},
    {62, "p64h32x4", v_patch<1, 64, 32, 4, 1, 1>, true},
    {63, "p64h32x4r2", v_patch<1, 64, 32, 4, 1, 2>, true},
    {64, "gb2<256,256>", v_gbig<256, 256, 4, 2, 2>, true},
    {65, "gb2<256,256>w128x64", v_gbig<256, 256, 2, 4, 2>, true},
    {66, "p64 two sets", v_patch2<64, 64, 8, 1>, true},
    {67, "chunk<128,64>", v_run<launch_chunk<128, 64, 4, 2>>},
    {68, "chunk<64,64>", v_run<launch_chunk<64, 64, 2, 4>>},
    {69, "chunk<256,64>", v_run<launch_chunk<256, 64, 4, 2>>},
    {70, "chunk<64,96>", v_run<launch_chunk<64, 96, 4, 2>>},
    {71, "chunk<128,96>", v_run<launch_chunk<128, 96, 4, 2>>},
    {72, "chunk<192,64>", v_run<launch_chunk<192, 64, 4, 2>>},
    {73, "chunk<256,96>", v_run<launch_chunk<256, 96, 4, 2>>},
    {74, "gbs<128,128>x2", v_gbig<128, 128, 2, 4, 2, 64, 2>, true},
    {75, "gbs<128,64>x2", v_gbig<128, 64, 2, 4, 2, 64, 2>, true},
    {76, "gbs<128,64>x3", v_gbig<128, 64, 2, 4, 2, 64, 3>, true},
    {77, "gbs<64,64>x4", v_gbig<64, 64, 2, 4, 2, 64, 4>, true},
    {78, "gbs<64,128>x3", v_gbig<64, 128, 2, 4, 2, 64, 3>, true},
    {79, "gbs<64,64>x2", v_gbig<64, 64, 2, 4, 2, 64, 2>, true},
    {80, "runp<256,64>", v_run<launch_run<256, 64, 4, 2, false, true>>},
    {81, "runp<256,128>", v_run<launch_run<256, 128, 4, 2, false, true>>},
    {82, "runp<224,128>", v_run<launch_run<224, 128, 2, 4, false, true>>},
    {83, "runp<320,64>", v_run<launch_run<320, 64, 4, 2, false, true>>},
    {84, "runp<192,128>", v_run<launch_run<192, 128, 4, 2, false, true>>},
    {85, "runp<128,64>", v_run<launch_run<128, 64, 2, 4, false, true>>},
    {86, "s2run<256,128>", v_run<launch_s2run<256, 128, 4, 2>, 2>},
    {87, "s2run<256,64>", v_run<launch_s2run<256, 64, 4, 2>, 2>},
    {88, "s2run<128,128>", v_run<launch_s2run<128, 128, 2, 4>, 2>},
    {89, "s2run<128,64>", v_run<launch_s2run<128, 64, 2, 4>, 2>},
#ifdef RVA_EXPERIMENTS
    {96, "run<256,128> nosel", v_run_nosel<256, 128, 4, 2>},
    {97, "run<256,64> nosel", v_run_nosel<256, 64, 4, 2>},
#endif
};

constexpr int kConvRows = (int)(sizeof kConvVariants / sizeof kConvVariants[0]);
#ifdef RVA_EXPERIMENTS
constexpr int RVA_CONV_VARIANTS = kConvRows - 3, kConvVariantsMax = 99;
#else
constexpr int RVA_CONV_VARIANTS = kConvRows - 1, kConvVariantsMax = RVA_CONV_VARIANTS;
#endif

constexpr bool conv_rows_numbered()
{
    for (int i = 0; i <= RVA_CONV_VARIANTS; ++i)
        if (kConvVariants[i].number != i) return false;
    return true;
}
static_assert(conv_rows_numbered(), "row i of kConvVariants carries variant number i: no gaps, no reordering");

const ConvVariant *find_variant(int variant)
{
    if (variant >= 0 && variant <= RVA_CONV_VARIANTS) return &kConvVariants[variant];
    for (int i = RVA_CONV_VARIANTS + 1; i < kConvRows; ++i)
        if (kConvVariants[i].number == variant) return &kConvVariants[i];
    return nullptr;
}

// ... 119 lines not shown
{
    if (!ctx) return RVA_ERR_ARG;
    if (!in || !weights || !bias || !out || batch <= 0 || H <= 0 || W <= 0 || Cin % 64 || Cout % 8 || ldi % 8 || nc % 8 ||
        (mode != 1 && mode != 2) || (mode == 1 && Cout != 64) || (mode == 2 && Cout != nc) ||
        ((uintptr_t)in | (uintptr_t)weights) % 16 || H > 2000 || W > 2000)
        return rva_fail(ctx, RVA_ERR_ARG, "rva_conv1x1_head_f16: unsupported shape (Cin %% 64; box branch Cout = 64; class branch Cout = nc)");
    ConvArgs a{};
    a.in = (const __half *)in; a.ldi = ldi; a.w = (const __half *)weights; a.bias = bias; a.out = nullptr; a.ldo = 0;
    a.H = H; a.W = W; a.Cin = Cin; a.CinPad = Cin; a.Cout = Cout; a.stride = 1; a.act = 0; a.Ho = H; a.Wo = W; a.M = batch * H * W;
    a.CoutPad = rva_ceil_div(Cout, 64) * 64; a.wy0 = 0; a.wrows = H;
    a.hout = (__half *)out; a.hmode = mode; a.hnc = nc; a.hA = anchors_total; a.ha0 = anchor_offset; a.hW = W; a.hHW = H * W;
    a.hstride = stride_px;
    a.hbox = boxes32;
    return launch_gather64_1x1<false, true>(ctx, "rva_conv1x1_head_f16", a, variant, (hipStream_t)stream_);
}

int rva_conv1x1_head_f16(rva_ctx *ctx, const void *in, int ldi, const void *weights, const float *bias, int batch, int H, int W,
                         int Cin, int Cout, int mode, void *out, int nc, int anchors_total, int anchor_offset, float stride_px,
                         int variant, rva_stream_t stream_)
{
    return conv1x1_head(ctx, in, ldi, weights, bias, batch, H, W, Cin, Cout, mode, out, nullptr, nc, anchors_total, anchor_offset, stride_px, variant, stream_);
}

int rva_conv1x1_head_box32_f16(rva_ctx *ctx, const void *in, int ldi, const void *weights, const float *bias, int batch, int H, int W,
                               int Cin, void *out, float *boxes32, int nc, int anchors_total, int anchor_offset, float stride_px,
                               int variant, rva_stream_t stream_)
{
    if (!ctx) return RVA_ERR_ARG;
    if (!boxes32 || (uintptr_t)boxes32 % 4 || anchor_offset < 0 || anchor_offset + H * W > anchors_total)
        return rva_fail(ctx, RVA_ERR_ARG, "rva_conv1x1_head_box32_f16: boxes32 must be a float tensor [batch, 4, anchors_total] and the level must lie inside it");
    return conv1x1_head(ctx, in, ldi, weights, bias, batch, H, W, Cin, 64, 1, out, boxes32, nc, anchors_total, anchor_offset, stride_px, variant, stream_);
}

int rva_conv_cout_pad(int Cout) { return rva_ceil_div(Cout, 64) * 64; }

int rva_conv_num_variants(void) { return kConvVariantsMax; }

const char *rva_conv_variant_name(int variant)
{
    const ConvVariant *row = find_variant(variant);
    return row ? row->name : nullptr;
}

int rva_stem_conv_f16(rva_ctx *ctx, const void *in_planar, const void *weights, const float *bias, void *out, int ldo,
                      int batch, int H, int W, int Cout, rva_stream_t stream_)
{
    if (!ctx || !in_planar || !weights || !bias || !out || Cout % 8 || Cout > 64 || ldo % 8)
        return rva_fail(ctx, RVA_ERR_ARG, "rva_stem_conv_f16: bad argument");
    StemArgs a{(const __half *)in_planar, nullptr, bias, (__half *)out, batch, H, W, (H - 1) / 2 + 1, (W - 1) / 2 + 1, Cout, ldo};
#ifdef RVA_ROW_STAMPS
    { const char *e = getenv("RVA_STEM_DBG"); a.dbg = e ? atoi(e) : 0; }
#endif
    const int total_tiles = rva_ceil_div(a.Wo, 32) * rva_ceil_div(a.Ho, 8) * batch;
    int grid = 256 * 4;
    if (grid > total_tiles) grid = total_tiles;
    if (W % 8 || ((uintptr_t)in_planar & 15)) return rva_fail(ctx, RVA_ERR_ARG, "rva_stem_conv_f16: W %% 8 == 0 and a 16-byte aligned input are required");
    k_stem<<<grid, 256, (size_t)(3 * 17 * 88 * 2) + (size_t)(256 * (Cout + 8 > LDSROW ? Cout + 8 : LDSROW) + 64 * LDSROW) * 2, (hipStream_t)stream_>>>(a, (const __half *)weights, bias);
    RVA_HIP(ctx, hipGetLastError());
    return RVA_OK;
}

int rva_c2f_pair32_f16(rva_ctx *ctx, const void *in, int ldi, const void *w1, const float *b1, const void *w2, const float *b2, void *out,
                       int ldo, int batch, int H, int W, rva_stream_t stream_)
{
    if (!ctx || !in || !w1 || !b1 || !w2 || !b2 || !out || batch <= 0 || H <= 0 || W <= 0 || ldi % 8 || ldo % 8 || ldi < 32 || ldo < 32)
        return rva_fail(ctx, RVA_ERR_ARG, "rva_c2f_pair32_f16: bad argument");
// ... 155 lines not shown
```

### realtime_video_analytics_32streams_amd/csrc/rva_internal.h

```cpp
#pragma once

#include <hip/hip_runtime.h>

#include <algorithm>
#include <cstdarg>
#include <cstdint>
#include <cstdio>
#include <map>
#include <string>
#include <vector>

#include "rva.h"

struct rva_resize_table {
    int32_t *ofs = nullptr;
    int16_t *w0 = nullptr;
    int16_t *w1 = nullptr;
    int n = 0;
};

struct rva_geom_cache {
    rva_resize_table x, y;
};

// ... 20 lines not shown
{
    char buf[512];
    va_list ap;
    va_start(ap, fmt);
    vsnprintf(buf, sizeof buf, fmt, ap);
    va_end(ap);
    if (ctx) ctx->err = buf;
    return code;
}

#define RVA_HIP(ctx, call)                                                                          \
    do {                                                                                            \
        hipError_t e_ = (call);                                                                     \
        if (e_ != hipSuccess)                                                                       \
            return rva_fail((ctx), RVA_ERR_HIP, "%s failed: %s (%s:%d)", #call, hipGetErrorString(e_), \
                            __FILE__, __LINE__);                                                    \
    } while (0)

int rva_get_taps(rva_ctx *ctx, int src, int dst, bool is_x, rva_resize_table *out);

static inline int rva_ceil_div(int a, int b) { return (a + b - 1) / b; }

hipError_t rva_func_smem(const void *fn, size_t bytes);

int rva_num_cus(rva_ctx *ctx);

bool rva_conv_variant_is_gather64(int variant);
bool rva_conv_variant_rows(int variant, int Cin, int ksize, int stride);

int rva_conv2d_nhwc_f16_sel(rva_ctx *ctx, const void *in, int ldi, const void *weights, const float *bias, void *out, int ldo,
                            const void *residual, int ldr, int batch, int sel_batch, int H, int W, int Cin, int Cout, int ksize, int stride,
                            int act, int variant, int y0, int y1, rva_stream_t stream);

void rva_jpeg_free(rva_ctx *ctx);

struct rva_dev_arena {
    std::vector<void *> allocs;

    int alloc(rva_ctx *ctx, float **dst, size_t n)
    {
        void *m = nullptr;
        RVA_HIP(ctx, hipMalloc(&m, std::max<size_t>(n, 1) * sizeof(float)));
        allocs.push_back(m);
        *dst = (float *)m;
        return RVA_OK;
    }

    int upload(rva_ctx *ctx, float **dst, const float *src, size_t n)
    {
        const int rc = alloc(ctx, dst, n);
        if (rc != RVA_OK) return rc;
        RVA_HIP(ctx, hipMemcpy(*dst, src, n * sizeof(float), hipMemcpyHostToDevice));
        return RVA_OK;
    }

    void release()
    {
        for (void *m : allocs) (void)hipFree(m);
        allocs.clear();
    }
};

int rva_clip_stem_prepare(rva_ctx *ctx);
int rva_clip_stem_launch(rva_ctx *ctx, const float *frames, const int32_t *frame_index, const float *w1, const float *b1, float *pooled,
                         int H, int W, int n_frames, hipStream_t st);
int rva_clip_mean_launch(rva_ctx *ctx, const float *partial, int tiles, float n, float *feat, int rows, int channels, hipStream_t st);
// ... 18 lines not shown
```

### realtime_video_analytics_32streams_amd/csrc/rva_plan.hip

```cpp
#include <cstring>
#include <memory>

#include "rva_internal.h"

namespace {

enum StepKind { K_CONV, K_UPCAT, K_HEAD, K_STEM2, K_STEM, K_SPPF3, K_POOL5, K_UP2, K_HEAD3, K_PAIR32,
                K_CONV_F32, K_STEM_F32, K_POOL5_F32, K_UP2_F32, K_HEAD_F32 };

struct View {
    char *base = nullptr; int ld = 0, off = 0, ch = 0, es = 2;
    void *ptr() const { return base + (size_t)es * off; }
    View sub(int o, int c) const { View v = *this; v.off += o; v.ch = c; return v; }
};

struct Step {
    StepKind kind;
    int lane = 0;
    int tunable = -1;
    const void *in = nullptr, *in2 = nullptr; int ldi = 0, ldi2 = 0, c_in = 0, c_in2 = 0;
    const void *w = nullptr, *w2 = nullptr; const float *b = nullptr, *b2 = nullptr;
    void *out = nullptr, *out2 = nullptr, *out3 = nullptr; int ldo = 0;
    const void *res = nullptr; int ldr = 0;
    int H = 0, W = 0, Cin = 0, Cout = 0, k = 0, stride = 0, act = 0, variant = 0;
    int mode = 0, a0 = 0; float stride_px = 0.f;
    int c_real = 0;
    int Ho = 0, y0 = 0, y1 = 0;
    const void *hb[3] = {nullptr, nullptr, nullptr}, *hk[3] = {nullptr, nullptr, nullptr};
    int32_t hldb[3] = {0, 0, 0}, hldc[3] = {0, 0, 0}, hh[3] = {0, 0, 0}, hw[3] = {0, 0, 0}; float hs[3] = {0, 0, 0};
};

struct Tunable { int step; std::string base, desc; };

}

struct rva_yolov8_plan {
    rva_ctx *ctx = nullptr;
    rva_yolov8_desc d{};
    int B = 0, H = 0, W = 0, nc = 0, A = 0;
    std::vector<void *> allocs;
    std::vector<Step> steps;
// ... 137 lines not shown
        s.c_real = cin_real;
        if (p->f32) {
            if (s.Cin % 16) return fail("fp32 plan: convolution input channels must be multiples of 16");
            push(s, "%d->%d k%ds%d %dx%d", cin_real, s.Cout, s.k, s.stride, h, w);
            return true;
        }
        if (s.Cin % 32 && !(p->d.flags & RVA_PLAN_NO_CIN_PAD)) s.Cin = (s.Cin + 31) / 32 * 32;
        push(s, "%d->%d k%ds%d %dx%d", cin_real, s.Cout, s.k, s.stride, h, w);
        return true;
    }
    bool conv1(const rva_conv_weights *c, View src, View dst, int h, int w, int act, const View *res = nullptr)
    {
        return c && conv(&c, 1, src, dst, h, w, act, res);
    }
    bool upcat(const rva_conv_weights *c, View low, View skip, View dst, int h, int w)
    {
        if (!c) return false;
        Step s{}; s.kind = K_UPCAT;
        if (!pack(&c, 1, &s.w, &s.b, &s.Cin, &s.Cout, &s.k, &s.stride)) return false;
        if (s.k != 1 || s.stride != 1 || s.Cin != low.ch + skip.ch || s.Cout != dst.ch) return fail("upsample + concat convolution does not fit");
        s.in = low.ptr(); s.ldi = low.ld; s.c_in = low.ch; s.in2 = skip.ptr(); s.ldi2 = skip.ld; s.c_in2 = skip.ch;
        s.out = dst.ptr(); s.ldo = dst.ld; s.H = h; s.W = w; s.act = 1;
        push(s, "up%d+%d->%d k1s1 %dx%d", low.ch, skip.ch, s.Cout, h, w);
        return true;
    }
    bool head(const rva_conv_weights *c, View src, int mode, int h, int w, int a0, float stride_px)
    {
        if (!c) return false;
        Step s{}; s.kind = K_HEAD;
        if (!pack(&c, 1, &s.w, &s.b, &s.Cin, &s.Cout, &s.k, &s.stride)) return false;
        if (s.k != 1 || s.stride != 1 || s.Cin != src.ch) return fail("head convolution does not fit");
        s.in = src.ptr(); s.ldi = src.ld; s.H = h; s.W = w; s.mode = mode; s.a0 = a0; s.stride_px = stride_px;
        push(s, "head%d:%d->%d k1s1 %dx%d", mode, s.Cin, s.Cout, h, w);
        return true;
    }
    bool c2f(int c1, int c2, int n, bool shortcut, const View *src, const View *low, const View *skip, View dst, int h, int w, const char *what)
    {
        const int c = c2 / 2;
        const long m = (long)p->B * h * w;
        const rva_conv_weights *cv1 = take(c1, 2 * c, 1, 1, what), *cv2 = take((2 + n) * c, c2, 1, 1, what);
        if (!cv1 || !cv2) return false;
        View cat = buf(m, (2 + n) * c);
        if (!cat.base) return false;
        if (low) { if (!upcat(cv1, *low, *skip, cat.sub(0, 2 * c), h, w)) return false; }
        else if (!conv1(cv1, *src, cat.sub(0, 2 * c), h, w, 1)) return false;
        for (int i = 0; i < n; ++i) {
            const rva_conv_weights *b1 = take(c, c, 3, 1, what), *b2 = take(c, c, 3, 1, what);
            View x = cat.sub((1 + i) * c, c);
            if (c == 32 && shortcut && !p->f32 && !(p->d.flags & RVA_PLAN_NO_PAIR32)) {
                Step s{}; s.kind = K_PAIR32;
                int ci, co, kk, st;
                if (!pack(&b1, 1, &s.w, &s.b, &ci, &co, &kk, &st) || !pack(&b2, 1, &s.w2, &s.b2, &ci, &co, &kk, &st)) return false;
                View y = cat.sub((2 + i) * c, c);
                s.in = x.ptr(); s.ldi = x.ld; s.out = y.ptr(); s.ldo = y.ld; s.H = h; s.W = w; s.Cin = s.Cout = c; s.k = 3; s.stride = 1; s.act = 1;
                push(s, nullptr);
                continue;
            }
            View tmp = buf(m, c);
            if (!tmp.base) return false;
            if (!conv1(b1, x, tmp, h, w, 1)) return false;
            if (!conv1(b2, tmp, cat.sub((2 + i) * c, c), h, w, 1, shortcut ? &x : nullptr)) return false;
        }
        return conv1(cv2, cat, dst, h, w, 1);
    }

    bool build()
// ... 104 lines not shown
        if (!conv1(take(c3, c3, 3, 2, "h16"), n3, cat18.sub(0, c3), h3, w3, 1)) return false;
        View m4 = buf((long)B * h4 * w4, c4);
        if (!m4.base || !c2f(c3 + c4, c4, nh, false, &cat18, nullptr, nullptr, m4, h4, w4, "h18")) return false;
        const int fork_m4 = (int)p->steps.size();
        if (!conv1(take(c4, c4, 3, 2, "h19"), m4, cat21.sub(0, c4), h4, w4, 1)) return false;
        View m5 = buf((long)B * h5 * w5, c5);
        if (!m5.base || !c2f(c4 + c5, c5, nh, false, &cat21, nullptr, nullptr, m5, h5, w5, "h21")) return false;
        const int rm4 = 4 * d.reg_max;
        int cb = c3 / 4 > rm4 ? c3 / 4 : rm4;
        if (cb < 16) cb = 16;
        int cc = c3 > (d.nc < 100 ? d.nc : 100) ? c3 : (d.nc < 100 ? d.nc : 100);
        p->A = h3 * w3 + h4 * w4 + h5 * w5;
        const rva_conv_weights *box[3][3], *cls[3][3];
        const int chs[3] = {c3, c4, c5};
        for (int l = 0; l < 3; ++l) {
            box[l][0] = take(chs[l], cb, 3, 1, "detect.box.0"); box[l][1] = take(cb, cb, 3, 1, "detect.box.1"); box[l][2] = take(cb, rm4, 1, 1, "detect.box.2");
            if (!box[l][0] || !box[l][1] || !box[l][2]) return false;
        }
        for (int l = 0; l < 3; ++l) {
            cls[l][0] = take(chs[l], cc, 3, 1, "detect.cls.0"); cls[l][1] = take(cc, cc, 3, 1, "detect.cls.1"); cls[l][2] = take(cc, d.nc, 1, 1, "detect.cls.2");
            if (!cls[l][0] || !cls[l][1] || !cls[l][2]) return false;
        }
        if (next != d.n_convs) return fail("convolution list longer than the architecture");
        p->fused_head = !p->f32 && cb % 64 == 0 && cc % 64 == 0 && rm4 == 64 && d.nc % 8 == 0;
        const View feats[3] = {n3, m4, m5};
        const int hs[3] = {h3, h4, h5}, ws[3] = {w3, w4, w5};
        const float strides[3] = {8.f, 16.f, 32.f};
        Step h3s{}; h3s.kind = K_HEAD3;
        int a0 = 0;
        for (int l = 0; l < 3; ++l) {
            lane = ((p->fused_head || p->f32) && l < 2) ? l + 1 : 0;
            if (lane) p->fork_step[lane] = l == 0 ? fork_n3 : fork_m4;
            const long m = (long)B * hs[l] * ws[l];
            View first = buf(m, cb + cc), b2 = buf(m, cb), k2 = buf(m, cc);
            if (!first.base || !b2.base || !k2.base) return false;
            const rva_conv_weights *sib[2] = {box[l][0], cls[l][0]};
            if (!conv(sib, 2, feats[l], first, hs[l], ws[l], 1)) return false;
            if (p->fused_head) {
                if (!conv1(box[l][1], first.sub(0, cb), b2, hs[l], ws[l], 1) || !head(box[l][2], b2, 1, hs[l], ws[l], a0, strides[l])) return false;
                if (!conv1(cls[l][1], first.sub(cb, cc), k2, hs[l], ws[l], 1) || !head(cls[l][2], k2, 2, hs[l], ws[l], a0, strides[l])) return false;
            } else {
                View bo = buf(m, rm4), ko = buf(m, d.nc);
                if (!bo.base || !ko.base) return false;
                if (!conv1(box[l][1], first.sub(0, cb), b2, hs[l], ws[l], 1) || !conv1(box[l][2], b2, bo, hs[l], ws[l], 0)) return false;
                if (!conv1(cls[l][1], first.sub(cb, cc), k2, hs[l], ws[l], 1) || !conv1(cls[l][2], k2, ko, hs[l], ws[l], 0)) return false;
                h3s.hb[l] = bo.ptr(); h3s.hldb[l] = bo.ld; h3s.hk[l] = ko.ptr(); h3s.hldc[l] = ko.ld; h3s.hh[l] = hs[l]; h3s.hw[l] = ws[l]; h3s.hs[l] = strides[l];
                if (p->f32) {
                    Step hs1{}; hs1.kind = K_HEAD_F32; hs1.in = bo.ptr(); hs1.ldi = bo.ld; hs1.in2 = ko.ptr(); hs1.ldi2 = ko.ld;
                    hs1.H = hs[l]; hs1.W = ws[l]; hs1.a0 = a0; hs1.stride_px = strides[l];
                    push(hs1, nullptr);
                }
            }
            a0 += hs[l] * ws[l];
        }
        lane = 0;
        if (!p->fused_head && !p->f32) push(h3s, nullptr);
        return err.empty();
    }
};

bool step_takes_rows(const Step &s, int variant)
{
    if (s.kind == K_STEM2) return true;
    return s.kind == K_CONV && rva_conv_variant_rows(variant, s.Cin, s.k, s.stride);
}

int launch_step(rva_yolov8_plan *p, const Step &s, int variant, const void *input, void *output, int n, rva_stream_t st, bool win)
{
    rva_ctx *c = p->ctx;
    if (win && (s.y0 > 0 || s.y1 < s.Ho) && step_takes_rows(s, variant)) {
        if (s.kind == K_STEM2) return rva_stem2_f16_rows(c, input, s.w, s.b, s.w2, s.b2, s.out, s.ldo, n, s.H, s.W, s.y0, s.y1, st);
        return rva_conv2d_nhwc_f16_sel(c, s.in, s.ldi, s.w, s.b, s.out, s.ldo, s.res, s.ldr, n, p->B, s.H, s.W, s.Cin, s.Cout, s.k, s.stride, s.act,
                                       variant, s.y0, s.y1, st);
    }
    if (p->box32 && output) {
        float *boxes = (float *)((char *)output + p->box_off);
        if (s.kind == K_HEAD && s.mode == 1)
            return rva_conv1x1_head_box32_f16(c, s.in, s.ldi, s.w, s.b, n, s.H, s.W, s.Cin, output, boxes, p->nc, p->A, s.a0, s.stride_px, variant, st);
        if (s.kind == K_HEAD3)
            return rva_yolo_head3_box32_f16(c, s.hb, s.hldb, s.hk, s.hldc, output, boxes, n, s.hh, s.hw, p->nc, p->A, s.hs, st);
    }
    switch (s.kind) {
    case K_CONV: return rva_conv2d_nhwc_f16_sel(c, s.in, s.ldi, s.w, s.b, s.out, s.ldo, s.res, s.ldr, n, p->B, s.H, s.W, s.Cin, s.Cout, s.k, s.stride, s.act, variant,
                                                0, -1, st);
    case K_UPCAT: return rva_conv1x1_upcat_f16(c, s.in, s.ldi, s.c_in, s.in2, s.ldi2, s.c_in2, s.w, s.b, s.out, s.ldo, n, s.H, s.W, s.Cout, s.act, variant, st);
    case K_HEAD: return rva_conv1x1_head_f16(c, s.in, s.ldi, s.w, s.b, n, s.H, s.W, s.Cin, s.Cout, s.mode, output, p->nc, p->A, s.a0, s.stride_px, variant, st);
    case K_PAIR32: return rva_c2f_pair32_f16(c, s.in, s.ldi, s.w, s.b, s.w2, s.b2, s.out, s.ldo, n, s.H, s.W, st);
    case K_STEM2: return rva_stem2_f16(c, input, s.w, s.b, s.w2, s.b2, s.out, s.ldo, n, s.H, s.W, st);
    case K_STEM: return rva_stem_conv_f16(c, input, s.w, s.b, s.out, s.ldo, n, s.H, s.W, s.Cout, st);
    case K_SPPF3: return rva_sppf_pool3_nhwc_f16(c, s.in, s.ldi, s.out, s.out2, s.out3, s.ldo, n, s.H, s.W, s.Cin, st);
    case K_POOL5: return rva_maxpool5_nhwc_f16(c, s.in, s.ldi, s.out, s.ldo, n, s.H, s.W, s.Cin, st);
    case K_UP2: return rva_upsample2x_nhwc_f16(c, s.in, s.ldi, s.out, s.ldo, n, s.H, s.W, s.Cin, st);
    case K_HEAD3: return rva_yolo_head3_f16(c, s.hb, s.hldb, s.hk, s.hldc, output, n, s.hh, s.hw, p->nc, p->A, s.hs, st);
    case K_CONV_F32: return rva_conv2d_nhwc_f32_v(c, s.in, s.ldi, s.w, s.b, s.out, s.ldo, s.res, s.ldr, n, s.H, s.W, s.Cin, s.Cout, s.k, s.stride, s.act, variant, st);
    case K_STEM_F32: return rva_stem_conv_f32(c, input, s.w, s.b, s.out, s.ldo, n, s.H, s.W, s.Cout, st);
    case K_POOL5_F32: return rva_maxpool5_nhwc_f32(c, s.in, s.ldi, s.out, s.ldo, n, s.H, s.W, s.Cin, st);
    case K_UP2_F32: return rva_upsample2x_nhwc_f32(c, s.in, s.ldi, s.out, s.ldo, n, s.H, s.W, s.Cin, st);
    case K_HEAD_F32: return rva_yolo_head_f32(c, s.in, s.ldi, s.in2, s.ldi2, output, n, s.H, s.W, p->nc, p->A, s.a0, s.stride_px, st);
    }
    return RVA_ERR_ARG;
}

bool variant_fits(const Step &s, int variant)
{
    if (s.kind == K_CONV) return variant >= 0;
    if (s.kind == K_CONV_F32) return variant >= 0 && variant <= rva_conv_f32_num_variants();
    return variant == 0 || rva_conv_variant_is_gather64(variant);
}

int out_rows(int H, int k, int stride) { return (H + 2 * (k / 2) - k) / stride + 1; }

void propagate_rows(rva_yolov8_plan *p)
{
    struct Slice { const char *lo, *hi; int H, y0, y1; };
    std::vector<Slice> written;
    const int es = p->f32 ? 4 : 2;
    const bool off = p->f32 || (p->rows_top <= 0 && p->rows_bottom >= p->H);
    auto read = [&](const void *ptr, int ch, int H, int *lo, int *hi) {
        const char *a = (const char *)ptr, *b = a + (size_t)ch * es;
        long covered = 0;
        int y0 = H, y1 = 0;
        for (const Slice &w : written) {
            const char *l = w.lo > a ? w.lo : a, *h = w.hi < b ? w.hi : b;
            if (l >= h) continue;
            if (w.H != H) return false;
            covered += h - l;
            if (w.y0 < y0) y0 = w.y0;
            if (w.y1 > y1) y1 = w.y1;
        }
        if (covered != b - a || y0 >= y1) return false;
        *lo = y0; *hi = y1;
        return true;
    };
    auto through = [](int k, int stride, int H, int *lo, int *hi) {
        int32_t a = 0, b = 0;
        (void)rva_conv_rows_through(k, stride, H, *lo, *hi, &a, &b);
        *lo = a; *hi = b;
        return out_rows(H, k, stride);
// ... 154 lines not shown
    if (total_bytes) *total_bytes = (int64_t)(p->box32 ? p->box_off + (size_t)p->B * 4 * p->A * 4 : head);
    if (boxes_offset) *boxes_offset = p->box32 ? (int64_t)p->box_off : -1;
    return RVA_OK;
}

int rva_yolov8_plan_tunable_desc(const rva_yolov8_plan *p, int index, char *buf, int len)
{
    if (!p || index < 0 || index >= (int)p->tunables.size() || !buf || len <= 0) return RVA_ERR_ARG;
    snprintf(buf, (size_t)len, "%s", p->tunables[index].desc.c_str());
    return RVA_OK;
}

int rva_yolov8_plan_set_variant(rva_yolov8_plan *p, int index, int variant)
{
    if (!p || index < 0 || index >= (int)p->tunables.size()) return RVA_ERR_ARG;
    Step &s = p->steps[p->tunables[index].step];
    if (!variant_fits(s, variant) || variant > rva_conv_num_variants()) return rva_fail(p->ctx, RVA_ERR_ARG, "rva_yolov8_plan_set_variant: variant %d does not exist for this layer", variant);
    p->primed = 0;
    s.variant = variant;
    return RVA_OK;
}

int rva_yolov8_plan_get_variant(const rva_yolov8_plan *p, int index)
{
    if (!p || index < 0 || index >= (int)p->tunables.size()) return -1;
    return p->steps[p->tunables[index].step].variant;
}

int rva_yolov8_plan_launch_tunable(rva_yolov8_plan *p, int index, int variant, void *output, rva_stream_t stream)
{
    if (!p || index < 0 || index >= (int)p->tunables.size()) return RVA_ERR_ARG;
    const Step &s = p->steps[p->tunables[index].step];
    if (!variant_fits(s, variant)) return RVA_ERR_ARG;
    if (s.kind == K_HEAD && !output) return RVA_ERR_ARG;
    return launch_step(p, s, variant, nullptr, output, p->B, stream, true);
}

int rva_yolov8_plan_run_range_n(rva_yolov8_plan *p, const void *input, void *output, int n, int first, int last, rva_stream_t stream)
{
    if (const int rc = check_run(p, input, output, n); rc != RVA_OK) return rc;
    if (first < 0 || last > (int)p->steps.size() || first > last) return RVA_ERR_ARG;
    return run_steps(p, input, output, n, first, last, stream, n <= p->primed);
}

int rva_yolov8_plan_run_range(rva_yolov8_plan *p, const void *input, void *output, int first, int last, rva_stream_t stream)
{
    return p ? rva_yolov8_plan_run_range_n(p, input, output, p->B, first, last, stream) : RVA_ERR_ARG;
}

int rva_yolov8_plan_run_n(rva_yolov8_plan *p, const void *input, void *output, int n, rva_stream_t stream)
{
    if (const int rc = check_run(p, input, output, n); rc != RVA_OK) return rc;
    const bool win = n <= p->primed;
    const int rc = run_steps(p, input, output, n, 0, (int)p->steps.size(), stream, win);
    if (rc == RVA_OK) note_complete_run(p, n, win, stream);
    return rc;
}

int rva_yolov8_plan_run(rva_yolov8_plan *p, const void *input, void *output, rva_stream_t stream)
{
    return p ? rva_yolov8_plan_run_n(p, input, output, p->B, stream) : RVA_ERR_ARG;
}

int rva_yolov8_plan_primed_images(const rva_yolov8_plan *p) { return p ? p->primed : 0; }

int rva_yolov8_plan_set_static_rows(rva_yolov8_plan *p, int top, int bottom)
{
// ... 65 lines not shown
```

### realtime_video_analytics_32streams_amd/detector.py

```python
from __future__ import annotations

import abc
import logging
from dataclasses import dataclass
from typing import Iterable, List, Optional, Sequence

import numpy as np
import torch

from . import _native as N
from . import ops
from .config import HIP_BACKENDS, TEMPORAL_MODELS, DetectorConfig
from .video_stream import FramePacket
from .yolov8 import build_detector_net, variant_from_path

LOGGER = logging.getLogger(__name__)


@dataclass(slots=True)
class Detection:

    stream_name: str
    frame_id: int
    class_id: int
# ... 122 lines not shown
                lb = res[1]
                self._note_rows(n, (int(lb.pad_top), int(lb.pad_top) + int(lb.new_h)) if key is not None else (0, self.input_hw[0]))
            return res
        dev = []
        for f in frames:
            t = torch.from_numpy(np.ascontiguousarray(f)) if isinstance(f, np.ndarray) else f
            dev.append(t.to(self.device, non_blocking=True).contiguous())
        self._in_border[n] = (None, 0)
        self._note_rows(n, (0, self.input_hw[0]))
        return ops.preprocess_bgr(dev, self.input_hw, self.half, out=self._in, ctx=self.ctx)

    def _note_rows(self, n, rows) -> None:
        rows = (max(rows[0], 0), min(rows[1], self.input_hw[0]))
        self._rows[n] = rows
        self._rows_told[n] = False

    def invalidate_engine(self) -> None:
        self._plans.clear()
        self._rows_told.clear()

    def plan_for(self, tensor: torch.Tensor):
        batch = int(tensor.shape[0])
        shape = (self._images(batch), int(tensor.shape[2]), int(tensor.shape[3]))
        key = shape if self._slot == 0 else shape + (self._slot,)
        plan = self._plans.get(key)
        if plan is None:
            from .engine import FusedYoloV8
            first = self._plans.get(shape) if self._slot else None
            n = shape[0] if self._slot == 0 else (shape[0], self._slot)
            rows = first.static_rows if first is not None else self._rows.get(n)
            plan = self._plans[key] = FusedYoloV8(self.net, shape[0], shape[1:], device=self.device, ctx=self.ctx,
                                                  autotune=first is None, tune_overlap=getattr(self, "tune_overlap", 1),
                                                  precision="fp32" if self.engine == "fused-f32" else "fp16", box_rows=self.box_rows,
                                                  static_rows=rows if self.engine == "fused" else None)
            if first is not None:
                plan.copy_tuning(first)
        plan.n = batch
        return plan

    def rows_pending(self, batch: int) -> bool:
        return not self._rows_told.get(self._buf_key(batch), True)

    def _tell_rows(self, plan, tensor: torch.Tensor) -> None:
        n = self._buf_key(int(tensor.shape[0]))
        own = self._in_bufs.get(n)
        if own is None or own.data_ptr() != tensor.data_ptr() or n not in self._rows:
            if plan.static_rows != (0, plan.H):
                plan.set_static_rows(0, plan.H)
                if n in self._rows:
                    self._rows_told[n] = False
            return
        if self._rows_told.get(n, True):
            return
        plan.set_static_rows(*self._rows[n])
        self._rows_told[n] = True

    def _infer(self, tensor: torch.Tensor):
        if self._infer_fn is not None:
            return self._infer_fn(tensor)
        if self.half:
            if tensor.dtype != torch.float16:
                raise TypeError("half detector: the fused plan takes the fp16 tensor K1 writes")
            plan = self.plan_for(tensor)
            if not torch.cuda.is_current_stream_capturing():
                self._tell_rows(plan, tensor)
            plan(tensor.contiguous())
            return plan.result()
        if self.engine == "fused-f32":
            if tensor.dtype != torch.float32:
                raise TypeError("fp32 plan: takes the fp32 tensor K1 writes for half=false")
            return self.plan_for(tensor)(tensor.contiguous())
# ... 60 lines not shown
```

### realtime_video_analytics_32streams_amd/engine.py

```python
from __future__ import annotations

import ctypes as C
import os
import time
from typing import Dict, List, Optional, Tuple

import numpy as np
import torch

from . import _native as N
from . import ops
from .yolov8 import C2f, ConvBnAct, YoloV8


_LIB_DIGEST: Optional[str] = None


def _lib_digest() -> str:
    global _LIB_DIGEST
    if _LIB_DIGEST is None:
        import hashlib
        _LIB_DIGEST = hashlib.sha256(N.LIB_PATH.read_bytes()).hexdigest()
    return _LIB_DIGEST


def _tuning_dir():
    import os
    from pathlib import Path
    d = os.environ.get("RVA_TUNE_CACHE_DIR")
    return Path(d) if d else Path(os.environ.get("XDG_CACHE_HOME", str(Path.home() / ".cache"))) / "rva_amd" / "autotune"


def module_order_convs(net: YoloV8) -> list:
    def c2f(m: C2f):
        out = [m.cv1, m.cv2]
        for b in m.m:
            out += [b.cv1, b.cv2]
        return out
    mods = [net.b0, net.b1, *c2f(net.b2), net.b3, *c2f(net.b4), net.b5, *c2f(net.b6), net.b7, *c2f(net.b8), net.b9.cv1, net.b9.cv2,
            *c2f(net.h12), *c2f(net.h15), net.h16, *c2f(net.h18), net.h19, *c2f(net.h21)]
    for branch in (net.detect.box, net.detect.cls):
        for seq in branch:
            mods += [seq[0], seq[1], seq[2]]
    return [m.conv if isinstance(m, ConvBnAct) else m for m in mods]


class _VariantCell:

    __slots__ = ("eng", "idx")

    def __init__(self, eng, idx):
        self.eng, self.idx = eng, idx

    def __getitem__(self, key):
        assert key == "variant"
        return int(self.eng.L.rva_yolov8_plan_get_variant(self.eng.handle, self.idx))

    def __setitem__(self, key, value):
        assert key == "variant"
        self.eng.ctx.check(self.eng.L.rva_yolov8_plan_set_variant(self.eng.handle, self.idx, int(value)), "rva_yolov8_plan_set_variant")


class FusedYoloV8:
    def __init__(self, net: YoloV8, batch: int, hw: Tuple[int, int] = (640, 640), device: Optional[torch.device] = None,
                 ctx: Optional[N.Context] = None, autotune: bool = True, tune_overlap: int = 1, precision: str = "fp16",
                 box_rows: str = "fp16", static_rows: Optional[Tuple[int, int]] = None):
        import os
        if precision not in ("fp16", "fp32"):
            raise ValueError(f"precision must be 'fp16' or 'fp32', not {precision!r}")
        if box_rows not in ("fp16", "fp32"):
            raise ValueError(f"box_rows must be 'fp16' or 'fp32', not {box_rows!r}")
        if box_rows == "fp32" and precision == "fp32":
            raise ValueError("box_rows='fp32' belongs to the fp16 plan: the output of precision='fp32' is fp32 already")
        self.box_rows = box_rows
        self.precision = precision
        self.f32 = precision == "fp32"
        self.tune_overlap = int(tune_overlap)
        self.ctx = ctx or ops.context()
        self.dev = device or torch.device("cuda", self.ctx.device)
        self.B, self.H, self.W = batch, hw[0], hw[1]
        self.n = batch
        assert hw[0] % 32 == 0 and hw[1] % 32 == 0
        net = net.fuse()
        self._net = net
        self.nc = net.nc
        self.L = N.lib()
        convs = module_order_convs(net)
        keep, arr = [], (N.ConvWeights * len(convs))()
        for i, c in enumerate(convs):
            w = np.ascontiguousarray(c.weight.detach().float().cpu().numpy())
            b = None if c.bias is None else np.ascontiguousarray(c.bias.detach().float().cpu().numpy())
            keep += [w, b]
            arr[i].weight = w.ctypes.data_as(C.POINTER(C.c_float))
            arr[i].bias = b.ctypes.data_as(C.POINTER(C.c_float)) if b is not None else None
            arr[i].cout, arr[i].cin, arr[i].k, arr[i].stride = int(w.shape[0]), int(w.shape[1]), int(w.shape[2]), int(c.stride[0])
        d = N.YoloV8Desc()
        d.batch, d.height, d.width = batch, hw[0], hw[1]
        d.widths[:] = [net.b0.conv.out_channels, net.b1.conv.out_channels, net.b3.conv.out_channels, net.b5.conv.out_channels,
                       net.b7.conv.out_channels]
        d.depth_backbone[:] = [len(net.b2.m), len(net.b4.m), len(net.b6.m), len(net.b8.m)]
        d.depth_head = len(net.h12.m)
        assert len(net.h15.m) == len(net.h18.m) == len(net.h21.m) == d.depth_head
        d.nc, d.reg_max, d.n_convs = net.nc, net.detect.reg_max, len(convs)
        d.flags = (N.RVA_PLAN_NO_STEM2 if os.environ.get("RVA_NO_STEM2", "0") == "1" else 0) | \
                  (N.RVA_PLAN_NO_CIN_PAD if os.environ.get("RVA_NO_CIN_PAD", "0") == "1" else 0) | \
                  (0 if self._use_pair32() else N.RVA_PLAN_NO_PAIR32) | \
                  (N.RVA_PLAN_F32 if self.f32 else 0) | (N.RVA_PLAN_BOX_F32 if box_rows == "fp32" else 0)
        h = C.c_void_p()
        with torch.cuda.device(self.dev):
            self.ctx.check(self.L.rva_yolov8_plan_create(self.ctx.handle, C.byref(d), arr, C.byref(h)), "rva_yolov8_plan_create")
        self.handle = h
        del keep
        self.static_rows = (0, self.H)
        self.rows_epoch = 0
        if static_rows is not None and tuple(static_rows) != (0, self.H) and os.environ.get("RVA_PLAN_NO_STATIC_ROWS") != "1":
            self.ctx.check(self.L.rva_yolov8_plan_set_static_rows(h, int(static_rows[0]), int(static_rows[1])), "rva_yolov8_plan_set_static_rows")
            self.static_rows = (int(static_rows[0]), int(static_rows[1]))
        info = [C.c_int32() for _ in range(5)]
        self.ctx.check(self.L.rva_yolov8_plan_info(h, *[C.byref(v) for v in info]), "rva_yolov8_plan_info")
        self.A, rows, self._n_steps, n_tun, self.quiet_step = (int(v.value) for v in info)
        assert rows == 4 + self.nc
        self.dtype = torch.float32 if self.f32 else torch.float16
        self.boxes32: Optional[torch.Tensor] = None
        self._boxes = {}
        if box_rows == "fp32":
            total, off = C.c_int64(), C.c_int64()
            self.ctx.check(self.L.rva_yolov8_plan_output_layout(h, C.byref(total), C.byref(off)), "rva_yolov8_plan_output_layout")
            self._out_layout = (int(total.value), int(off.value))
            self.out, self.boxes32 = self._alloc_split()
            self._boxes[0] = self.boxes32
        else:
            self.out = torch.empty((batch, rows, self.A), dtype=self.dtype, device=self.dev)
        self._outs = {0: self.out}
        self.fused_stem = not self.f32 and not (d.flags & N.RVA_PLAN_NO_STEM2) and tuple(d.widths[:2]) == (32, 64)
        self._n_tunable = n_tun
        self._read_tunables()
        self._side = None
        self._forks = bool(self.fused_head_lanes())
        self.concurrent_heads = os.environ.get("RVA_SERIAL_HEADS") != "1"
        if autotune:
# ... 32 lines not shown

    def _alloc_split(self) -> Tuple[torch.Tensor, torch.Tensor]:
        total, off = self._out_layout
        rows = 4 + self.nc
        buf = torch.empty((total,), dtype=torch.uint8, device=self.dev)
        head = buf[:self.B * rows * self.A * 2].view(torch.float16).view(self.B, rows, self.A)
        boxes = buf[off:off + self.B * 4 * self.A * 4].view(torch.float32).view(self.B, 4, self.A)
        return head, boxes

    def fused_head_lanes(self) -> bool:
        return self.f32 or any(d.startswith("head1:") for _, _, d in self._tunable)

    def __del__(self):
        try:
            if getattr(self, "handle", None):
                self.L.rva_yolov8_plan_destroy(self.handle)
                self.handle = None
        except Exception:
            pass

    def _tuning_key(self) -> str:
        import hashlib
        import os
        h = hashlib.sha256()
        h.update(torch.cuda.get_device_name(self.dev).encode())
        h.update(_lib_digest().encode())
        h.update(repr((self.B, self.H, self.W, [d for _, _, d in self._tunable])).encode())
        h.update(b"per-layer times; in-plan pass opt-in, three overlapping passes")
        h.update(repr([os.environ.get(k, "") for k in ("RVA_SKIP_VARIANTS", "RVA_TUNE_IN_PLAN", "RVA_TUNE_OVERLAP", "RVA_TUNE_TOP",
                                                       "RVA_TUNE_WITHIN", "RVA_NO_STEM2", "RVA_HEAD_SPLIT", "RVA_NO_CIN_PAD")]).encode())
        h.update(repr(int(os.environ.get("RVA_TUNE_LAYER_OVERLAP", getattr(self, "tune_overlap", 1)))).encode())
        if getattr(self, "f32", False):
            h.update(b"precision fp32")
        return h.hexdigest()[:24]

    def _load_tuning(self) -> bool:
        import json
        f = _tuning_dir() / f"{self._tuning_key()}.json"
        try:
            rec = json.loads(f.read_text())
            picks = rec["variants"]
            if len(picks) != len(self._tunable) or any(d != pd for (_, _, d), (pd, _) in zip(self._tunable, picks)):
                return False
        except (OSError, ValueError, KeyError, TypeError):
            return False
        try:
            for (_, state, _), (_, v) in zip(self._tunable, picks):
                state["variant"] = int(v)
        except RuntimeError:
            for _, state, _ in self._tunable:
                state["variant"] = 0
            return False
        self.tuning = [tuple(t) for t in rec.get("tuning", [])]
        self.tuning_source = str(f)
        return True

    def _store_tuning(self) -> None:
        import json
        import os
        d = _tuning_dir()
        try:
            d.mkdir(parents=True, exist_ok=True)
            tmp = d / f".{self._tuning_key()}.{os.getpid()}.tmp"
            tmp.write_text(json.dumps({"device": torch.cuda.get_device_name(self.dev), "batch": self.B, "hw": [self.H, self.W],
                                       "variants": [[desc, st["variant"]] for _, st, desc in self._tunable],
                                       "tuning": [list(t) for t in self.tuning]}))
# ... 55 lines not shown
                if us < best[1]:
                    best = (variant, us)
            state["variant"] = best[0]
            cache[desc] = best
            self._candidates[desc] = sorted(timed)[:int(os.environ.get('RVA_TUNE_TOP', '5'))]
            self.tuning.append((desc, best[0], round(best[1], 1)))
        if os.environ.get("RVA_TUNE_IN_PLAN", "0") == "1":
            self._refine_in_plan()
        if use_cache:
            self._store_tuning()

    def copy_tuning(self, other: "FusedYoloV8") -> None:
        assert len(self._tunable) == len(other._tunable) and self.precision == other.precision
        for (_, mine, d1), (_, theirs, d2) in zip(self._tunable, other._tunable):
            assert d1 == d2
            mine["variant"] = theirs["variant"]
        self.tuning = list(getattr(other, "tuning", []))
        self.tuning_source = "copied from the first slot's plan"

    def _refine_in_plan(self, reps: int = 12, within: float = 1.25) -> None:
        import os
        within = float(os.environ.get('RVA_TUNE_WITHIN', within))
        """Second pass of the kernel selection, on the real objective: a layer's launch time in isolation is not its cost inside
        the plan -- the detect branches run on side streams beside the neck, and a kernel that wants every CU for itself (one
        128-KB workgroup per CU) shares worse than a two-workgroups-per-CU one that is a few per cent slower alone.  For the
        layers with runners-up within 25 % the whole forward pass is timed with each candidate (coordinate descent, most
        expensive layers first) and a candidate is kept when the pass gets faster by more than the timing noise."""
        x = torch.zeros((self.B, 3, self.H, self.W), dtype=self.dtype, device=self.dev)
        twins: list = []
        lanes = self.concurrent_heads
        n_over = int(os.environ.get("RVA_TUNE_OVERLAP", "3"))
        if n_over >= 2:
            twins = [FusedYoloV8(self._net, self.B, (self.H, self.W), device=self.dev, ctx=self.ctx, autotune=False, precision=self.precision,
                                 box_rows=self.box_rows, static_rows=self.static_rows)
                     for _ in range(n_over - 1)]
            from .ops import chain_streams
            streams = chain_streams(self.dev, n_over)
            self.concurrent_heads = False
            for t in twins:
                t.concurrent_heads = False

        def forward_us() -> float:
            best = float("inf")
            for t in twins:
                t.copy_tuning(self)
            group = [self] + twins
            rounds = max(reps // len(group), 2)
            for _ in range(2):
                torch.cuda.synchronize()
                t0 = time.perf_counter()
                if not twins:
                    for _ in range(reps):
                        self(x)
                else:
                    for _ in range(rounds):
                        for pl, st in zip(group, streams):
                            with torch.cuda.stream(st):
                                pl(x)
                torch.cuda.synchronize()
                best = min(best, (time.perf_counter() - t0) / (rounds * len(group) if twins else reps) * 1e6)
            return best
        by_desc: Dict[str, list] = {}
        for _, state, desc in self._tunable:
            by_desc.setdefault(desc, []).append(state)
        cost = {d: v[0][0] * len(by_desc[d]) for d, v in self._candidates.items() if v}
        order = [d for d in sorted(cost, key=cost.get, reverse=True)
                 if len(self._candidates[d]) > 1 and self._candidates[d][1][0] <= within * self._candidates[d][0][0]][:24]
# ... 83 lines not shown
```

Before: 24070.

## Fuse detect-head 1x1 conv and box/cls decode into the 3x3 conv epilogue

Adds a tail to the 3x3 conv kernels (big, run, chunk variants). After the 3x3 output tile is staged in LDS, the tail applies the final 1x1 head conv with MFMA and then does the DFL box decode or sigmoid class decode, writing directly to the detection output. This removes the intermediate 3x3 output buffer round trip through global memory and two extra kernel launches per branch per level. The new path is enabled by default for the fused fp16 engine. The cost is more register and LDS pressure in the conv kernels, and fewer tile variants can be used, since the tail requires Cout and Cout2 to fit in a single BN tile.

```diff
diff --git a/include/rva.h b/include/rva.h
--- a/include/rva.h
+++ b/include/rva.h
@@ -160,6 +160,10 @@
 int rva_conv1x1_head_box32_f16(rva_ctx *ctx, const void *in, int ldi, const void *weights, const float *bias, int batch,
                                int H, int W, int Cin, void *out, float *boxes32, int nc, int anchors_total, int anchor_offset,
                                float stride_px, int variant, rva_stream_t stream);
+int rva_conv3x3_head_f16_v(rva_ctx *ctx, const void *in, int ldi, const void *weights3, const float *bias3, const void *weights1,
+                           const float *bias1, int batch, int H, int W, int Cin, int Cmid, int mode, int nc, void *out,
+                           float *boxes32, int anchors_total, int anchor_offset, float stride_px, int variant, rva_stream_t stream);
+int rva_conv_variant_tail(int variant, int Cmid);
 int rva_stem_conv_f16(rva_ctx *ctx, const void *in_planar, const void *weights, const float *bias,
                       void *out, int ldo, int batch, int H, int W, int Cout, rva_stream_t stream);
 
@@ -209,6 +213,8 @@
 #define RVA_PLAN_NO_PAIR32 4
 #define RVA_PLAN_F32 8
 #define RVA_PLAN_BOX_F32 16
+#define RVA_PLAN_TAIL_BOX(l) (32 << (l))
+#define RVA_PLAN_TAIL_CLS(l) (256 << (l))
 typedef struct rva_yolov8_plan rva_yolov8_plan;
 typedef struct rva_yolov8_desc {
     int32_t batch, height, width;
diff --git a/realtime_video_analytics_32streams_amd/_native.py b/realtime_video_analytics_32streams_amd/_native.py
--- a/realtime_video_analytics_32streams_amd/_native.py
+++ b/realtime_video_analytics_32streams_amd/_native.py
@@ -82,6 +82,17 @@
 RVA_PLAN_NO_PAIR32 = 4
 RVA_PLAN_F32 = 8
 RVA_PLAN_BOX_F32 = 16
+
+
+def RVA_PLAN_TAIL_BOX(level: int) -> int:
+    return 32 << level
+
+
+def RVA_PLAN_TAIL_CLS(level: int) -> int:
+    return 256 << level
+
+
+RVA_PLAN_TAIL_ALL = sum(RVA_PLAN_TAIL_BOX(l) | RVA_PLAN_TAIL_CLS(l) for l in range(3))
 
 
 def _stale() -> bool:
@@ -193,6 +204,8 @@
         "rva_conv2d_nhwc_f16_rows": (C.c_int, [_P, _P, C.c_int, _P, _P, _P, C.c_int, _P, C.c_int] + [C.c_int] * 11 + [_P]),
         "rva_conv_rows_through": (C.c_int, [C.c_int] * 5 + [i32p, i32p]),
         "rva_stem2_f16_rows": (C.c_int, [_P, _P, _P, _P, _P, _P, _P, C.c_int, C.c_int, C.c_int, C.c_int, C.c_int, C.c_int, _P]),
+        "rva_conv3x3_head_f16_v": (C.c_int, [_P, _P, C.c_int, _P, _P, _P, _P] + [C.c_int] * 7 + [_P, _P, C.c_int, C.c_int, C.c_float, C.c_int, _P]),
+        "rva_conv_variant_tail": (C.c_int, [C.c_int, C.c_int]),
         "rva_stem_conv_f16": (C.c_int, [_P, _P, _P, _P, _P, C.c_int, C.c_int, C.c_int, C.c_int, C.c_int, _P]),
         "rva_stem2_f16": (C.c_int, [_P, _P, _P, _P, _P, _P, _P, C.c_int, C.c_int, C.c_int, C.c_int, _P]),
         "rva_c2f_pair32_f16": (C.c_int, [_P, _P, C.c_int, _P, _P, _P, _P, _P, C.c_int, C.c_int, C.c_int, C.c_int, _P]),
@@ -318,6 +331,7 @@
     "rva_resnet_plan_run", "rva_resnet_plan_run_post", "rva_resnet_plan_stage", "rva_resnet_f16_plan_create", "rva_resnet_f16_plan_destroy",
     "rva_resnet_f16_plan_info", "rva_resnet_f16_plan_run", "rva_resnet_f16_plan_run_post", "rva_resnet_f16_plan_stage", "rva_jpeg_max_bytes", "rva_jpeg_encode_bgr", "rva_jpeg_status",
     "rva_jpeg_batch_create", "rva_jpeg_batch_destroy", "rva_jpeg_batch_encode", "rva_preview_nv12_batch",
+    "rva_conv3x3_head_f16_v", "rva_conv_variant_tail",
 ]
 
 
diff --git a/realtime_video_analytics_32streams_amd/csrc/rva_conv.hip b/realtime_video_analytics_32streams_amd/csrc/rva_conv.hip
--- a/realtime_video_analytics_32streams_amd/csrc/rva_conv.hip
+++ b/realtime_video_analytics_32streams_amd/csrc/rva_conv.hip
@@ -1052,6 +1052,137 @@
     }
 }
 
+struct HeadOut {
+    __half *hout; float *hbox;
+    int hnc, hA, ha0, hW; float hstride;
+};
+
+__device__ __forceinline__ void head_box_row(const HeadOut &h, const __half *row, int b, int i)
+{
+    __half *o = h.hout + (size_t)b * (4 + h.hnc) * h.hA + h.ha0 + i;
+    float d[4];
+#pragma unroll
+    for (int sd = 0; sd < 4; ++sd) {
+        float v[16], mx = -1e30f;
+        const uint4 q0 = *reinterpret_cast<const uint4 *>(row + sd * 16), q1 = *reinterpret_cast<const uint4 *>(row + sd * 16 + 8);
+        const __half2 *h0 = reinterpret_cast<const __half2 *>(&q0), *h1 = reinterpret_cast<const __half2 *>(&q1);
+#pragma unroll
+        for (int t = 0; t < 4; ++t) {
+            float2 f = __half22float2(h0[t]); v[2 * t] = f.x; v[2 * t + 1] = f.y;
+            f = __half22float2(h1[t]); v[8 + 2 * t] = f.x; v[9 + 2 * t] = f.y;
+        }
+#pragma unroll
+        for (int t = 0; t < 16; ++t) mx = fmaxf(mx, v[t]);
+        float se = 0.f, sw = 0.f;
+#pragma unroll
+        for (int t = 0; t < 16; ++t) { const float e = __expf(v[t] - mx); se += e; sw += e * (float)t; }
+        d[sd] = sw / se;
+    }
+    const float ax = (float)(i % h.hW) + 0.5f, ay = (float)(i / h.hW) + 0.5f;
+    const float x1 = ax - d[0], y1 = ay - d[1], x2 = ax + d[2], y2 = ay + d[3];
+    o[0] = __float2half_rn((x1 + x2) * 0.5f * h.hstride);
+    o[(size_t)h.hA] = __float2half_rn((y1 + y2) * 0.5f * h.hstride);
+    o[(size_t)2 * h.hA] = __float2half_rn((x2 - x1) * h.hstride);
+    o[(size_t)3 * h.hA] = __float2half_rn((y2 - y1) * h.hstride);
+    if (h.hbox) {
+        float *o32 = h.hbox + (size_t)b * 4 * h.hA + h.ha0 + i;
+        o32[0] = (x1 + x2) * 0.5f * h.hstride;
+        o32[(size_t)h.hA] = (y1 + y2) * 0.5f * h.hstride;
+        o32[(size_t)2 * h.hA] = (x2 - x1) * h.hstride;
+        o32[(size_t)3 * h.hA] = (y2 - y1) * h.hstride;
+    }
+}
+
+__device__ __forceinline__ void head_cls8(const HeadOut &h, const __half *row8, int b, int i, int c)
+{
+    __half *o = h.hout + (size_t)b * (4 + h.hnc) * h.hA + h.ha0 + i;
+    const uint4 q = *reinterpret_cast<const uint4 *>(row8);
+    const __half2 *hq = reinterpret_cast<const __half2 *>(&q);
+#pragma unroll
+    for (int t = 0; t < 4; ++t) {
+        const float2 f = __half22float2(hq[t]);
+        o[(size_t)(4 + c + 2 * t) * h.hA] = __float2half_rn(__builtin_amdgcn_rcpf(1.0f + __expf(-f.x)));
+        o[(size_t)(5 + c + 2 * t) * h.hA] = __float2half_rn(__builtin_amdgcn_rcpf(1.0f + __expf(-f.y)));
+    }
+}
+
+struct TailArgs {
+    const __half *w2;
+    const float *b2;
+    int Cout2, hmode, hHW;
+    HeadOut h;
+};
+template <class G> struct WithTail : G { TailArgs t; };
+template <class G, bool TAIL> struct TailSel { typedef G type; };
+template <class G> struct TailSel<G, true> { typedef WithTail<G> type; };
+
+template <int BM, int BN, bool PADO, int NFPMAX = 5>
+__device__ __forceinline__ void conv3_head_tail(const TailArgs &t, __half *stage, const int *rowmap, int P0, int M, int Cmid, int tid)
+{
+    static_assert(BM % 16 == 0 && BN % 32 == 0, "whole fragments");
+    constexpr int SROW = BN + 8, KBMAX = BN / 32;
+    constexpr int NFP = BN / 16 < NFPMAX ? BN / 16 : NFPMAX;
+    const int lane = tid & 63, wv = __builtin_amdgcn_readfirstlane(tid >> 6);
+    const int kbn = Cmid >> 5, nf2 = (t.Cout2 + 15) >> 4;
+    const __half *wlane = t.w2 + (size_t)(lane & 15) * Cmid + (lane >> 4) * 8;
+    h8 wf[NFP][KBMAX];
+    float4 bvp[NFP];
+#pragma unroll
+    for (int i = 0; i < NFP; ++i)
+        if (i < nf2) {
+#pragma unroll
+            for (int kb = 0; kb < KBMAX; ++kb)
+                if (kb < kbn) wf[i][kb] = *reinterpret_cast<const h8 *>(wlane + (size_t)(16 * i) * Cmid + kb * 32);
+            bvp[i] = *reinterpret_cast<const float4 *>(t.b2 + 16 * i + (lane >> 4) * 4);
+        }
+    __syncthreads();
+    for (int f = wv; f < BM / 16; f += 8) {
+        __half *prow = stage + (size_t)(f * 16 + (lane & 15)) * SROW;
+        h8 bf[KBMAX];
+#pragma unroll
+        for (int kb = 0; kb < KBMAX; ++kb)
+            if (kb < kbn) bf[kb] = *reinterpret_cast<const h8 *>(prow + kb * 32 + (lane >> 4) * 8);
+        auto put = [&](int i, const f4 &acc, const float4 &bv) {
+            const float v0 = acc[0] + bv.x, v1 = acc[1] + bv.y, v2 = acc[2] + bv.z, v3 = acc[3] + bv.w;
+            __half2 lo = __floats2half2_rn(v0, v1), hi = __floats2half2_rn(v2, v3);
+            uint2 pk;
+            pk.x = *reinterpret_cast<uint32_t *>(&lo);
+            pk.y = *reinterpret_cast<uint32_t *>(&hi);
+            *reinterpret_cast<uint2 *>(prow + 16 * i + (lane >> 4) * 4) = pk;
+        };
+#pragma unroll
+        for (int i = 0; i < NFP; ++i)
+            if (i < nf2) {
+                f4 acc = f4{0.f, 0.f, 0.f, 0.f};
+#pragma unroll
+                for (int kb = 0; kb < KBMAX; ++kb)
+                    if (kb < kbn) acc = __builtin_amdgcn_mfma_f32_16x16x32_f16(wf[i][kb], bf[kb], acc, 0, 0, 0);
+                put(i, acc, bvp[i]);
+            }
+        for (int i = NFP; i < nf2; ++i) {
+            f4 acc = f4{0.f, 0.f, 0.f, 0.f};
+#pragma unroll
+            for (int kb = 0; kb < KBMAX; ++kb)
+                if (kb < kbn) {
+                    const h8 af = *reinterpret_cast<const h8 *>(wlane + (size_t)(16 * i) * Cmid + kb * 32);
+                    acc = __builtin_amdgcn_mfma_f32_16x16x32_f16(af, bf[kb], acc, 0, 0, 0);
+                }
+            put(i, acc, *reinterpret_cast<const float4 *>(t.b2 + 16 * i + (lane >> 4) * 4));
+        }
+    }
+    __syncthreads();
+    const int groups = t.hmode == 1 ? 1 : t.Cout2 >> 3;
+    for (int q = tid; q < BM * groups; q += 512) {
+        const int g = q / BM, r = q - g * BM;
+        const int m = PADO ? rowmap[r] : P0 + r;
+        if (PADO ? m < 0 : m >= M) continue;
+        const int b = m / t.hHW, i = m - b * t.hHW;
+        const __half *row = stage + (size_t)r * SROW;
+        if (t.hmode == 1) head_box_row(t.h, row, b, i);
+        else head_cls8(t.h, row + g * 8, b, i, g * 8);
+    }
+}
+
 struct BigArgs {
     const __half *in; int ldi;
     const __half *w; const float *bias;
@@ -1104,8 +1235,8 @@
     }
 }
 
-template <int BM, int BN, int WGM, int WGN, int NSLOT>
-__global__ void __launch_bounds__(512) __attribute__((amdgpu_waves_per_eu(NSLOT == 2 ? 4 : 2))) k_conv3_big(BigArgs a)
+template <int BM, int BN, int WGM, int WGN, int NSLOT, bool TAIL = false>
+__global__ void __launch_bounds__(512) __attribute__((amdgpu_waves_per_eu(NSLOT == 2 ? 4 : 2))) k_conv3_big(typename TailSel<BigArgs, TAIL>::type a)
 {
     static_assert(WGM * WGN == 8, "eight waves");
     static_assert(NSLOT == 2 || NSLOT == 3, "ring depth");
@@ -1301,6 +1432,10 @@
             *reinterpret_cast<uint2 *>(stage + (size_t)px * SROW + co) = pk;
         }
     }
+    if constexpr (TAIL) {
+        conv3_head_tail<BM, BN, false, (NSLOT == 2 && BN == 128 && BM > 128) ? 3 : 5>(a.t, stage, nullptr, P0, a.M, a.Cout, tid);
+        return;
+    }
     __syncthreads();
     constexpr int CPR = BN / 8;
 #pragma unroll 4
@@ -1330,8 +1465,11 @@
 #undef BIG_ISSUE_ADVANCE
 #undef BIG_ISSUE_PIECE
 
-template <int BM, int BN, int WGM, int WGN, int NSLOT>
-hipError_t launch_big(BigArgs &a, hipStream_t s)
+template <int BN, class G>
+bool tail_fits(const G &a) { return a.Cout % 32 == 0 && a.Cout <= BN && a.t.Cout2 % 8 == 0 && a.t.Cout2 <= BN && !a.res; }
+
+template <int BM, int BN, int WGM, int WGN, int NSLOT, bool TAIL = false>
+hipError_t launch_big(typename TailSel<BigArgs, TAIL>::type &a, hipStream_t s)
 {
     constexpr size_t ring = (size_t)NSLOT * ((BM + 2 + 15) / 16 + 3 * BN / 16) * 1024;
     constexpr size_t st = (size_t)BM * (BN + 8) * 2;
@@ -1339,10 +1477,11 @@
     static_assert(smem <= 160 * 1024, "LDS budget");
     if (a.Cin % 32 || a.CoutPad % 4 || a.M >= (1 << 24)) return hipErrorInvalidValue;
     if ((size_t)a.M * a.ldi * 2 >= (1ull << 32) || (size_t)a.CoutPad * 9 * a.Cin * 2 >= (1ull << 32)) return hipErrorInvalidValue;
-    if (hipError_t e = rva_func_smem((const void *)k_conv3_big<BM, BN, WGM, WGN, NSLOT>, smem); e != hipSuccess) return e;
+    if constexpr (TAIL) if (!tail_fits<BN>(a)) return hipErrorInvalidValue;
+    if (hipError_t e = rva_func_smem((const void *)k_conv3_big<BM, BN, WGM, WGN, NSLOT, TAIL>, smem); e != hipSuccess) return e;
     a.n_tiles = rva_ceil_div(a.Cout, BN);
     a.m_tiles = rva_ceil_div(a.M, BM);
-    k_conv3_big<BM, BN, WGM, WGN, NSLOT><<<rva_ceil_div(a.m_tiles, 8) * 8 * a.n_tiles, 512, smem, s>>>(a);
+    k_conv3_big<BM, BN, WGM, WGN, NSLOT, TAIL><<<rva_ceil_div(a.m_tiles, 8) * 8 * a.n_tiles, 512, smem, s>>>(a);
     return hipGetLastError();
 }
 
@@ -1354,8 +1493,8 @@
     int H, W, Cin, Cout, CoutPad, act, n_tiles, M, m_tiles, apieces, map_off;
 };
 
-template <int BM, int BN, int WGM, int WGN, bool NOSEL = false, bool PADO = false>
-__global__ void __launch_bounds__(512) __attribute__((amdgpu_waves_per_eu(BN <= 64 && BM <= 320 ? 4 : 2))) k_conv3_run(RunArgs a)
+template <int BM, int BN, int WGM, int WGN, bool NOSEL = false, bool PADO = false, bool TAIL = false>
+__global__ void __launch_bounds__(512) __attribute__((amdgpu_waves_per_eu(BN <= 64 && BM <= 320 ? 4 : 2))) k_conv3_run(typename TailSel<RunArgs, TAIL>::type a)
 {
     static_assert(WGM * WGN == 8, "eight waves");
     constexpr int TM = BM / WGM, TN = BN / WGN, FM = TM / 16, FN = TN / 16;
@@ -1545,6 +1684,10 @@
             *reinterpret_cast<uint2 *>(stage + (size_t)px * SROW + co) = pk;
         }
     }
+    if constexpr (TAIL) {
+        conv3_head_tail<BM, BN, PADO>(a.t, stage, rowmap, P0, a.M, a.Cout, tid);
+        return;
+    }
     __syncthreads();
     constexpr int CPR = BN / 8;
 #pragma unroll 4
@@ -1570,8 +1713,8 @@
     STAMP(6);
 }
 
-template <int BM, int BN, int WGM, int WGN, bool NOSEL = false, bool PADO = false>
-hipError_t launch_run(RunArgs &a, hipStream_t s)
+template <int BM, int BN, int WGM, int WGN, bool NOSEL = false, bool PADO = false, bool TAIL = false>
+hipError_t launch_run(typename TailSel<RunArgs, TAIL>::type &a, hipStream_t s)
 {
     if (a.Cin % 32 || a.CoutPad % 4 || a.W > 160 || a.M >= (1 << 24)) return hipErrorInvalidValue;
     if ((size_t)a.M * a.ldi * 2 >= (1ull << 32) || (size_t)a.CoutPad * 9 * a.Cin * 2 >= (1ull << 32)) return hipErrorInvalidValue;
@@ -1590,10 +1733,11 @@
         smem += (size_t)BM * 4;
     }
     if (smem > 160 * 1024) return hipErrorInvalidValue;
-    if (hipError_t e = rva_func_smem((const void *)k_conv3_run<BM, BN, WGM, WGN, NOSEL, PADO>, 160 * 1024); e != hipSuccess) return e;
+    if constexpr (TAIL) if (!tail_fits<BN>(a)) return hipErrorInvalidValue;
+    if (hipError_t e = rva_func_smem((const void *)k_conv3_run<BM, BN, WGM, WGN, NOSEL, PADO, TAIL>, 160 * 1024); e != hipSuccess) return e;
     a.n_tiles = rva_ceil_div(a.Cout, BN);
     a.m_tiles = (int)((mp + BM - 1) / BM);
-    k_conv3_run<BM, BN, WGM, WGN, NOSEL, PADO><<<rva_ceil_div(a.m_tiles, 8) * 8 * a.n_tiles, 512, smem, s>>>(a);
+    k_conv3_run<BM, BN, WGM, WGN, NOSEL, PADO, TAIL><<<rva_ceil_div(a.m_tiles, 8) * 8 * a.n_tiles, 512, smem, s>>>(a);
     return hipGetLastError();
 }
 
@@ -1785,8 +1929,8 @@
     return hipGetLastError();
 }
 
-template <int BM, int BN, int WGM, int WGN>
-__global__ void __launch_bounds__(512) __attribute__((amdgpu_waves_per_eu(2))) k_conv3_chunk(RunArgs a)
+template <int BM, int BN, int WGM, int WGN, bool TAIL = false>
+__global__ void __launch_bounds__(512) __attribute__((amdgpu_waves_per_eu(2))) k_conv3_chunk(typename TailSel<RunArgs, TAIL>::type a)
 {
     static_assert(WGM * WGN == 8, "eight waves");
     constexpr int TM = BM / WGM, TN = BN / WGN, FM = TM / 16, FN = TN / 16;
@@ -1926,6 +2070,10 @@
             *reinterpret_cast<uint2 *>(stage + (size_t)px * SROW + co) = pk;
         }
     }
+    if constexpr (TAIL) {
+        conv3_head_tail<BM, BN, false>(a.t, stage, nullptr, P0, a.M, a.Cout, tid);
+        return;
+    }
     __syncthreads();
     constexpr int CPR = BN / 8;
 #pragma unroll 4
@@ -1950,8 +2098,8 @@
     }
 }
 
-template <int BM, int BN, int WGM, int WGN>
-hipError_t launch_chunk(RunArgs &a, hipStream_t s)
+template <int BM, int BN, int WGM, int WGN, bool TAIL = false>
+hipError_t launch_chunk(typename TailSel<RunArgs, TAIL>::type &a, hipStream_t s)
 {
     if (a.Cin % 32 || a.CoutPad % 4 || a.W > 160 || a.M >= (1 << 24)) return hipErrorInvalidValue;
     if ((size_t)a.M * a.ldi * 2 >= (1ull << 32) || (size_t)a.CoutPad * 9 * a.Cin * 2 >= (1ull << 32)) return hipErrorInvalidValue;
@@ -1961,10 +2109,11 @@
     const size_t st = (size_t)BM * (BN + 8) * 2;
     const size_t smem = ring > st ? ring : st;
     if (smem > 160 * 1024) return hipErrorInvalidValue;
-    if (hipError_t e = rva_func_smem((const void *)k_conv3_chunk<BM, BN, WGM, WGN>, 160 * 1024); e != hipSuccess) return e;
+    if constexpr (TAIL) if (!tail_fits<BN>(a)) return hipErrorInvalidValue;
+    if (hipError_t e = rva_func_smem((const void *)k_conv3_chunk<BM, BN, WGM, WGN, TAIL>, 160 * 1024); e != hipSuccess) return e;
     a.n_tiles = rva_ceil_div(a.Cout, BN);
     a.m_tiles = rva_ceil_div(a.M, BM);
-    k_conv3_chunk<BM, BN, WGM, WGN><<<rva_ceil_div(a.m_tiles, 8) * 8 * a.n_tiles, 512, smem, s>>>(a);
+    k_conv3_chunk<BM, BN, WGM, WGN, TAIL><<<rva_ceil_div(a.m_tiles, 8) * 8 * a.n_tiles, 512, smem, s>>>(a);
     return hipGetLastError();
 }
 
@@ -2163,56 +2312,17 @@
     }
     __syncthreads();
     if constexpr (HEAD) {
+        const HeadOut h{a.hout, a.hbox, a.hnc, a.hA, a.ha0, a.hW, a.hstride};
         for (int r = tid; r < BM; r += 512) {
             const int m = P0 + r;
             if (m >= a.M) continue;
             const int b = m / a.hHW, i = m - b * a.hHW;
-            __half *o = a.hout + (size_t)b * (4 + a.hnc) * a.hA + a.ha0 + i;
             const __half *row = stage + (size_t)r * SROW;
             if (a.hmode == 1) {
-                float d[4];
-#pragma unroll
-                for (int sd = 0; sd < 4; ++sd) {
-                    float v[16], mx = -1e30f;
-                    const uint4 q0 = *reinterpret_cast<const uint4 *>(row + sd * 16), q1 = *reinterpret_cast<const uint4 *>(row + sd * 16 + 8);
-                    const __half2 *h0 = reinterpret_cast<const __half2 *>(&q0), *h1 = reinterpret_cast<const __half2 *>(&q1);
-#pragma unroll
-                    for (int t = 0; t < 4; ++t) {
-                        float2 f = __half22float2(h0[t]); v[2 * t] = f.x; v[2 * t + 1] = f.y;
-                        f = __half22float2(h1[t]); v[8 + 2 * t] = f.x; v[9 + 2 * t] = f.y;
-                    }
-#pragma unroll
-                    for (int t = 0; t < 16; ++t) mx = fmaxf(mx, v[t]);
-                    float se = 0.f, sw = 0.f;
-#pragma unroll
-                    for (int t = 0; t < 16; ++t) { const float e = __expf(v[t] - mx); se += e; sw += e * (float)t; }
-                    d[sd] = sw / se;
-                }
-                const float ax = (float)(i % a.hW) + 0.5f, ay = (float)(i / a.hW) + 0.5f;
-                const float x1 = ax - d[0], y1 = ay - d[1], x2 = ax + d[2], y2 = ay + d[3];
-                o[0] = __float2half_rn((x1 + x2) * 0.5f * a.hstride);
-                o[(size_t)a.hA] = __float2half_rn((y1 + y2) * 0.5f * a.hstride);
-                o[(size_t)2 * a.hA] = __float2half_rn((x2 - x1) * a.hstride);
-                o[(size_t)3 * a.hA] = __float2half_rn((y2 - y1) * a.hstride);
-                if (a.hbox) {
-                    float *o32 = a.hbox + (size_t)b * 4 * a.hA + a.ha0 + i;
-                    o32[0] = (x1 + x2) * 0.5f * a.hstride;
-                    o32[(size_t)a.hA] = (y1 + y2) * 0.5f * a.hstride;
-                    o32[(size_t)2 * a.hA] = (x2 - x1) * a.hstride;
-                    o32[(size_t)3 * a.hA] = (y2 - y1) * a.hstride;
-                }
+                head_box_row(h, row, b, i);
             } else {
                 const int cend = min(BN, a.Cout - n0);
-                for (int c = 0; c < cend; c += 8) {
-                    const uint4 q = *reinterpret_cast<const uint4 *>(row + c);
-                    const __half2 *hq = reinterpret_cast<const __half2 *>(&q);
-#pragma unroll
-                    for (int t = 0; t < 4; ++t) {
-                        const float2 f = __half22float2(hq[t]);
-                        o[(size_t)(4 + n0 + c + 2 * t) * a.hA] = __float2half_rn(__builtin_amdgcn_rcpf(1.0f + __expf(-f.x)));
-                        o[(size_t)(5 + n0 + c + 2 * t) * a.hA] = __float2half_rn(__builtin_amdgcn_rcpf(1.0f + __expf(-f.y)));
-                    }
-                }
+                for (int c = 0; c < cend; c += 8) head_cls8(h, row + c, b, i, n0 + c);
             }
         }
         return;
@@ -3207,6 +3317,38 @@
 }
 #endif
 
+struct TailCall { ConvCall c; TailArgs t; };
+
+template <class G>
+WithTail<G> tail_args(const TailCall &tc)
+{
+    WithTail<G> g{};
+    static_cast<G &>(g) = dma3_args<G>(tc.c);
+    g.t = tc.t;
+    return g;
+}
+
+template <int BM, int BN, int WGM, int WGN, int NSLOT>
+hipError_t t_big(const TailCall &tc)
+{
+    WithTail<BigArgs> g = tail_args<BigArgs>(tc);
+    return launch_big<BM, BN, WGM, WGN, NSLOT, true>(g, tc.c.s);
+}
+
+template <int BM, int BN, int WGM, int WGN, bool PADO>
+hipError_t t_run(const TailCall &tc)
+{
+    WithTail<RunArgs> g = tail_args<RunArgs>(tc);
+    return launch_run<BM, BN, WGM, WGN, false, PADO, true>(g, tc.c.s);
+}
+
+template <int BM, int BN, int WGM, int WGN>
+hipError_t t_chunk(const TailCall &tc)
+{
+    WithTail<RunArgs> g = tail_args<RunArgs>(tc);
+    return launch_chunk<BM, BN, WGM, WGN, true>(g, tc.c.s);
+}
+
 hipError_t launch_variant(int variant, const ConvCall &c);
 
 inline bool auto_picks_gather(int Cin, int ksize, int stride) { return Cin % 64 == 0 && ((ksize == 3 && stride == 2) || (ksize == 1 && stride == 1)); }
@@ -3278,6 +3420,8 @@
     const char *name;
     hipError_t (*launch)(const ConvCall &);
     bool rows = false;
+    hipError_t (*tail)(const TailCall &) = nullptr;
+    int tail_bn = 0;
 };
 
 constexpr ConvVariant kConvVariants[] = {
@@ -3302,18 +3446,18 @@
     {18, "row2<64,32>", v_row<64, 32, true>},
     {19, "row2<128,64>", v_row<128, 64, true>},
     {20, "row2<128,32>", v_row<128, 32, true>},
-    {21, "big<256,128>", v_big<256, 128, 4, 2, 3>},
-    {22, "big<128,128>", v_big<128, 128, 2, 4, 3>},
-    {23, "big<256,64>", v_big<256, 64, 4, 2, 3>},
-    {24, "big<128,64>", v_big<128, 64, 2, 4, 3>},
-    {25, "big2<192,128>", v_big<192, 128, 4, 2, 2>},
-    {26, "big2<128,128>", v_big<128, 128, 2, 4, 2>},
-    {27, "big2<256,64>", v_big<256, 64, 4, 2, 2>},
-    {28, "big2<128,64>", v_big<128, 64, 2, 4, 2>},
-    {29, "big2<224,128>", v_big<224, 128, 2, 4, 2>},
-    {30, "big2<160,128>", v_big<160, 128, 2, 4, 2>},
-    {31, "big2<384,64>", v_big<384, 64, 8, 1, 2>},
-    {32, "big2<320,64>", v_big<320, 64, 4, 2, 2>},
+    {21, "big<256,128>", v_big<256, 128, 4, 2, 3>, false, t_big<256, 128, 4, 2, 3>, 128},
+    {22, "big<128,128>", v_big<128, 128, 2, 4, 3>, false, t_big<128, 128, 2, 4, 3>, 128},
+    {23, "big<256,64>", v_big<256, 64, 4, 2, 3>, false, t_big<256, 64, 4, 2, 3>, 64},
+    {24, "big<128,64>", v_big<128, 64, 2, 4, 3>, false, t_big<128, 64, 2, 4, 3>, 64},
+    {25, "big2<192,128>", v_big<192, 128, 4, 2, 2>, false, t_big<192, 128, 4, 2, 2>, 128},
+    {26, "big2<128,128>", v_big<128, 128, 2, 4, 2>, false, t_big<128, 128, 2, 4, 2>, 128},
+    {27, "big2<256,64>", v_big<256, 64, 4, 2, 2>, false, t_big<256, 64, 4, 2, 2>, 64},
+    {28, "big2<128,64>", v_big<128, 64, 2, 4, 2>, false, t_big<128, 64, 2, 4, 2>, 64},
+    {29, "big2<224,128>", v_big<224, 128, 2, 4, 2>, false, t_big<224, 128, 2, 4, 2>, 128},
+    {30, "big2<160,128>", v_big<160, 128, 2, 4, 2>, false, t_big<160, 128, 2, 4, 2>, 128},
+    {31, "big2<384,64>", v_big<384, 64, 8, 1, 2>, false, t_big<384, 64, 8, 1, 2>, 64},
+    {32, "big2<320,64>", v_big<320, 64, 4, 2, 2>, false, t_big<320, 64, 4, 2, 2>, 64},
 #define RVA_ROW(n, name, ...) {n, name, v_gbig<__VA_ARGS__>, true},
     RVA_GATHER64_TILES(RVA_ROW)
 #undef RVA_ROW
@@ -3329,27 +3473,27 @@
     {49, "p64x8db", v_patch<1, 64, 64, 8, 2>, true},
     {50, "p64x4r2db", v_patch<1, 64, 64, 4, 2, 2>, true},
     {51, "p64x8r2", v_patch<1, 64, 64, 8, 1, 2>, true},
-    {52, "run<256,64>", v_run<launch_run<256, 64, 4, 2>>},
-    {53, "run<128,64>", v_run<launch_run<128, 64, 2, 4>>},
-    {54, "run<384,64>", v_run<launch_run<384, 64, 8, 1>>},
-    {55, "run<192,128>", v_run<launch_run<192, 128, 4, 2>>},
-    {56, "run<256,128>", v_run<launch_run<256, 128, 4, 2>>},
-    {57, "run<128,128>", v_run<launch_run<128, 128, 2, 4>>},
-    {58, "run<224,128>", v_run<launch_run<224, 128, 2, 4>>},
-    {59, "run<160,128>", v_run<launch_run<160, 128, 2, 4>>},
-    {60, "run<320,64>", v_run<launch_run<320, 64, 4, 2>>},
+    {52, "run<256,64>", v_run<launch_run<256, 64, 4, 2>>, false, t_run<256, 64, 4, 2, false>, 64},
+    {53, "run<128,64>", v_run<launch_run<128, 64, 2, 4>>, false, t_run<128, 64, 2, 4, false>, 64},
+    {54, "run<384,64>", v_run<launch_run<384, 64, 8, 1>>, false, t_run<384, 64, 8, 1, false>, 64},
+    {55, "run<192,128>", v_run<launch_run<192, 128, 4, 2>>, false, t_run<192, 128, 4, 2, false>, 128},
+    {56, "run<256,128>", v_run<launch_run<256, 128, 4, 2>>, false, t_run<256, 128, 4, 2, false>, 128},
+    {57, "run<128,128>", v_run<launch_run<128, 128, 2, 4>>, false, t_run<128, 128, 2, 4, false>, 128},
+    {58, "run<224,128>", v_run<launch_run<224, 128, 2, 4>>, false, t_run<224, 128, 2, 4, false>, 128},
+    {59, "run<160,128>", v_run<launch_run<160, 128, 2, 4>>, false, t_run<160, 128, 2, 4, false>, 128},
+    {60, "run<320,64>", v_run<launch_run<320, 64, 4, 2>>, false, t_run<320, 64, 4, 2, false>, 64},
     {61, "p64h32x8", v_patch<1, 64, 32, 8, 1, 1>, true},
     {62, "p64h32x4", v_patch<1, 64, 32, 4, 1, 1>, true},
     {63, "p64h32x4r2", v_patch<1, 64, 32, 4, 1, 2>, true},
     {64, "gb2<256,256>", v_gbig<256, 256, 4, 2, 2>, true},
     {65, "gb2<256,256>w128x64", v_gbig<256, 256, 2, 4, 2>, true},
     {66, "p64 two sets", v_patch2<64, 64, 8, 1>, true},
-    {67, "chunk<128,64>", v_run<launch_chunk<128, 64, 4, 2>>},
-    {68, "chunk<64,64>", v_run<launch_chunk<64, 64, 2, 4>>},
-    {69, "chunk<256,64>", v_run<launch_chunk<256, 64, 4, 2>>},
+    {67, "chunk<128,64>", v_run<launch_chunk<128, 64, 4, 2>>, false, t_chunk<128, 64, 4, 2>, 64},
+    {68, "chunk<64,64>", v_run<launch_chunk<64, 64, 2, 4>>, false, t_chunk<64, 64, 2, 4>, 64},
+    {69, "chunk<256,64>", v_run<launch_chunk<256, 64, 4, 2>>, false, t_chunk<256, 64, 4, 2>, 64},
     {70, "chunk<64,96>", v_run<launch_chunk<64, 96, 4, 2>>},
     {71, "chunk<128,96>", v_run<launch_chunk<128, 96, 4, 2>>},
-    {72, "chunk<192,64>", v_run<launch_chunk<192, 64, 4, 2>>},
+    {72, "chunk<192,64>", v_run<launch_chunk<192, 64, 4, 2>>, false, t_chunk<192, 64, 4, 2>, 64},
     {73, "chunk<256,96>", v_run<launch_chunk<256, 96, 4, 2>>},
     {74, "gbs<128,128>x2", v_gbig<128, 128, 2, 4, 2, 64, 2>, true},
     {75, "gbs<128,64>x2", v_gbig<128, 64, 2, 4, 2, 64, 2>, true},
@@ -3357,12 +3501,12 @@
     {77, "gbs<64,64>x4", v_gbig<64, 64, 2, 4, 2, 64, 4>, true},
     {78, "gbs<64,128>x3", v_gbig<64, 128, 2, 4, 2, 64, 3>, true},
     {79, "gbs<64,64>x2", v_gbig<64, 64, 2, 4, 2, 64, 2>, true},
-    {80, "runp<256,64>", v_run<launch_run<256, 64, 4, 2, false, true>>},
-    {81, "runp<256,128>", v_run<launch_run<256, 128, 4, 2, false, true>>},
-    {82, "runp<224,128>", v_run<launch_run<224, 128, 2, 4, false, true>>},
-    {83, "runp<320,64>", v_run<launch_run<320, 64, 4, 2, false, true>>},
-    {84, "runp<192,128>", v_run<launch_run<192, 128, 4, 2, false, true>>},
-    {85, "runp<128,64>", v_run<launch_run<128, 64, 2, 4, false, true>>},
+    {80, "runp<256,64>", v_run<launch_run<256, 64, 4, 2, false, true>>, false, t_run<256, 64, 4, 2, true>, 64},
+    {81, "runp<256,128>", v_run<launch_run<256, 128, 4, 2, false, true>>, false, t_run<256, 128, 4, 2, true>, 128},
+    {82, "runp<224,128>", v_run<launch_run<224, 128, 2, 4, false, true>>, false, t_run<224, 128, 2, 4, true>, 128},
+    {83, "runp<320,64>", v_run<launch_run<320, 64, 4, 2, false, true>>, false, t_run<320, 64, 4, 2, true>, 64},
+    {84, "runp<192,128>", v_run<launch_run<192, 128, 4, 2, false, true>>, false, t_run<192, 128, 4, 2, true>, 128},
+    {85, "runp<128,64>", v_run<launch_run<128, 64, 2, 4, false, true>>, false, t_run<128, 64, 2, 4, true>, 64},
     {86, "s2run<256,128>", v_run<launch_s2run<256, 128, 4, 2>, 2>},
     {87, "s2run<256,64>", v_run<launch_s2run<256, 64, 4, 2>, 2>},
     {88, "s2run<128,128>", v_run<launch_s2run<128, 128, 2, 4>, 2>},
@@ -3548,6 +3692,67 @@
     return conv1x1_head(ctx, in, ldi, weights, bias, batch, H, W, Cin, 64, 1, out, boxes32, nc, anchors_total, anchor_offset, stride_px, variant, stream_);
 }
 
+}
+
+static int tail_auto_pick(int Cmid, long selM)
+{
+    return rva_conv_cout_pad(Cmid) % 128 == 0 ? (selM * Cmid >= 20000000L ? 25 : 21) : (selM >= 100000 ? 31 : 23);
+}
+
+int rva_conv3x3_head_f16_sel(rva_ctx *ctx, const void *in, int ldi, const void *w3, const float *b3, const void *w1, const float *b1,
+                             int batch, int sel_batch, int H, int W, int Cin, int Cmid, int mode, int nc, void *out, float *boxes32,
+                             int anchors_total, int anchor_offset, float stride_px, int variant, rva_stream_t stream_)
+{
+    if (!rva_conv_variant_tail(variant, Cmid))
+        return ctx ? rva_fail(ctx, RVA_ERR_ARG, "rva_conv3x3_head_f16_v: variant %d has no head tail for %d channels", variant, Cmid) : RVA_ERR_ARG;
+    if (!ctx) return RVA_ERR_ARG;
+    const int Cout2 = mode == 1 ? 64 : nc;
+    if (!in || !w3 || !b3 || !w1 || !b1 || !out || batch <= 0 || sel_batch < batch || H <= 0 || W <= 0 || Cin % 8 || ldi % 8 || nc <= 0 || nc % 8 ||
+        (mode != 1 && mode != 2) || (mode == 2 && boxes32) || ((uintptr_t)in | (uintptr_t)w3 | (uintptr_t)w1) % 16 || (uintptr_t)boxes32 % 4 ||
+        anchor_offset < 0 || anchor_offset + H * W > anchors_total)
+        return rva_fail(ctx, RVA_ERR_ARG, "rva_conv3x3_head_f16_v: unsupported shape/alignment (Cin %% 8, ld %% 8, nc %% 8, mode 1 / 2, boxes32 with "
+                                          "mode 1 only, the level inside anchors_total)");
+    TailCall tc{};
+    ConvCall &c = tc.c;
+    ConvArgs &a = c.a;
+    a.in = (const __half *)in; a.ldi = ldi; a.w = (const __half *)w3; a.bias = b3; a.out = nullptr; a.ldo = 0; a.res = nullptr; a.ldr = 0;
+    a.H = H; a.W = W; a.Cin = Cin; a.CinPad = rva_ceil_div(Cin, 32) * 32; a.Cout = Cmid; a.stride = 1; a.act = 1;
+    a.Ho = H; a.Wo = W; a.M = batch * H * W; a.wy0 = 0; a.wrows = H;
+    c.y0 = 0; c.y1 = H; c.batch = batch; c.sel_batch = sel_batch; c.ksize = 3;
+    c.cpad = rva_conv_cout_pad(Cmid);
+    c.num_cus = rva_num_cus(ctx);
+    c.s = (hipStream_t)stream_;
+    tc.t.w2 = (const __half *)w1; tc.t.b2 = b1; tc.t.Cout2 = Cout2; tc.t.hmode = mode; tc.t.hHW = H * W;
+    tc.t.h = HeadOut{(__half *)out, boxes32, nc, anchors_total, anchor_offset, W, stride_px};
+    if (variant == 0) {
+        variant = tail_auto_pick(Cmid, (long)sel_batch * H * W);
+        if (!first_choice_fits(c, variant)) return rva_fail(ctx, RVA_ERR_ARG, "rva_conv3x3_head_f16_v: the tensors are too large for variant 0's tile");
+    }
+    const hipError_t ev = find_variant(variant)->tail(tc);
+    if (ev == hipSuccess) return RVA_OK;
+    (void)hipGetLastError();
+    if (ev == hipErrorInvalidValue) return rva_fail(ctx, RVA_ERR_ARG, "rva_conv3x3_head_f16_v: variant %d not applicable here", variant);
+    return rva_fail(ctx, RVA_ERR_HIP, "rva_conv3x3_head_f16_v: variant %d: launch failed: %s", variant, hipGetErrorString(ev));
+}
+
+extern "C" {
+
+int rva_conv3x3_head_f16_v(rva_ctx *ctx, const void *in, int ldi, const void *w3, const float *b3, const void *w1, const float *b1,
+                           int batch, int H, int W, int Cin, int Cmid, int mode, int nc, void *out, float *boxes32, int anchors_total,
+                           int anchor_offset, float stride_px, int variant, rva_stream_t stream_)
+{
+    return rva_conv3x3_head_f16_sel(ctx, in, ldi, w3, b3, w1, b1, batch, batch, H, W, Cin, Cmid, mode, nc, out, boxes32, anchors_total,
+                                    anchor_offset, stride_px, variant, stream_);
+}
+
+int rva_conv_variant_tail(int variant, int Cmid)
+{
+    if (Cmid <= 0 || Cmid % 32) return 0;
+    if (variant == 0) variant = tail_auto_pick(Cmid, 0);
+    const ConvVariant *row = find_variant(variant);
+    return row && row->tail && row->tail_bn >= Cmid;
+}
+
 int rva_conv_cout_pad(int Cout) { return rva_ceil_div(Cout, 64) * 64; }
 
 int rva_conv_num_variants(void) { return kConvVariantsMax; }
diff --git a/realtime_video_analytics_32streams_amd/csrc/rva_internal.h b/realtime_video_analytics_32streams_amd/csrc/rva_internal.h
--- a/realtime_video_analytics_32streams_amd/csrc/rva_internal.h
+++ b/realtime_video_analytics_32streams_amd/csrc/rva_internal.h
@@ -76,6 +76,10 @@
                             const void *residual, int ldr, int batch, int sel_batch, int H, int W, int Cin, int Cout, int ksize, int stride,
                             int act, int variant, int y0, int y1, rva_stream_t stream);
 
+int rva_conv3x3_head_f16_sel(rva_ctx *ctx, const void *in, int ldi, const void *w3, const float *b3, const void *w1, const float *b1,
+                             int batch, int sel_batch, int H, int W, int Cin, int Cmid, int mode, int nc, void *out, float *boxes32,
+                             int anchors_total, int anchor_offset, float stride_px, int variant, rva_stream_t stream);
+
 void rva_jpeg_free(rva_ctx *ctx);
 
 struct rva_dev_arena {
diff --git a/realtime_video_analytics_32streams_amd/csrc/rva_plan.hip b/realtime_video_analytics_32streams_amd/csrc/rva_plan.hip
--- a/realtime_video_analytics_32streams_amd/csrc/rva_plan.hip
+++ b/realtime_video_analytics_32streams_amd/csrc/rva_plan.hip
@@ -6,7 +6,8 @@
 namespace {
 
 enum StepKind { K_CONV, K_UPCAT, K_HEAD, K_STEM2, K_STEM, K_SPPF3, K_POOL5, K_UP2, K_HEAD3, K_PAIR32,
-                K_CONV_F32, K_STEM_F32, K_POOL5_F32, K_UP2_F32, K_HEAD_F32 };
+                K_CONV_F32, K_STEM_F32, K_POOL5_F32, K_UP2_F32, K_HEAD_F32,
+                K_CONV_HEAD };
 
 struct View {
     char *base = nullptr; int ld = 0, off = 0, ch = 0, es = 2;
@@ -210,6 +211,23 @@
         if (s.k != 1 || s.stride != 1 || s.Cin != src.ch) return fail("head convolution does not fit");
         s.in = src.ptr(); s.ldi = src.ld; s.H = h; s.W = w; s.mode = mode; s.a0 = a0; s.stride_px = stride_px;
         push(s, "head%d:%d->%d k1s1 %dx%d", mode, s.Cin, s.Cout, h, w);
+        return true;
+    }
+    static bool tail_covers(int cmid)
+    {
+        for (int v = 0; v <= rva_conv_num_variants(); ++v)
+            if (rva_conv_variant_tail(v, cmid)) return true;
+        return false;
+    }
+    bool conv_head(const rva_conv_weights *c3, const rva_conv_weights *c1, View src, int mode, int h, int w, int a0, float stride_px)
+    {
+        if (!c3 || !c1) return false;
+        Step s{}; s.kind = K_CONV_HEAD;
+        int ci, co, kk, st;
+        if (!pack(&c3, 1, &s.w, &s.b, &s.Cin, &s.Cout, &s.k, &s.stride) || !pack(&c1, 1, &s.w2, &s.b2, &ci, &co, &kk, &st)) return false;
+        if (s.k != 3 || s.stride != 1 || s.Cin != src.ch || s.Cin % 32 || kk != 1 || st != 1 || ci != s.Cout) return fail("head tail does not fit");
+        s.in = src.ptr(); s.ldi = src.ld; s.H = h; s.W = w; s.act = 1; s.mode = mode; s.a0 = a0; s.stride_px = stride_px; s.c_real = s.Cin;
+        push(s, "head%d:%d->%d k3s1+%d->%d k1s1 %dx%d", mode, s.Cin, s.Cout, ci, co, h, w);
         return true;
     }
     bool c2f(int c1, int c2, int n, bool shortcut, const View *src, const View *low, const View *skip, View dst, int h, int w, const char *what)
@@ -380,13 +398,17 @@
             lane = ((p->fused_head || p->f32) && l < 2) ? l + 1 : 0;
             if (lane) p->fork_step[lane] = l == 0 ? fork_n3 : fork_m4;
             const long m = (long)B * hs[l] * ws[l];
-            View first = buf(m, cb + cc), b2 = buf(m, cb), k2 = buf(m, cc);
-            if (!first.base || !b2.base || !k2.base) return false;
+            const bool tail_b = p->fused_head && (d.flags & RVA_PLAN_TAIL_BOX(l)) && cb % 32 == 0 && tail_covers(cb);
+            const bool tail_k = p->fused_head && (d.flags & RVA_PLAN_TAIL_CLS(l)) && cc % 32 == 0 && tail_covers(cc);
+            View first = buf(m, cb + cc), b2 = tail_b ? View{} : buf(m, cb), k2 = tail_k ? View{} : buf(m, cc);
+            if (!first.base || (!tail_b && !b2.base) || (!tail_k && !k2.base)) return false;
             const rva_conv_weights *sib[2] = {box[l][0], cls[l][0]};
             if (!conv(sib, 2, feats[l], first, hs[l], ws[l], 1)) return false;
             if (p->fused_head) {
-                if (!conv1(box[l][1], first.sub(0, cb), b2, hs[l], ws[l], 1) || !head(box[l][2], b2, 1, hs[l], ws[l], a0, strides[l])) return false;
-                if (!conv1(cls[l][1], first.sub(cb, cc), k2, hs[l], ws[l], 1) || !head(cls[l][2], k2, 2, hs[l], ws[l], a0, strides[l])) return false;
+                if (tail_b) { if (!conv_head(box[l][1], box[l][2], first.sub(0, cb), 1, hs[l], ws[l], a0, strides[l])) return false; }
+                else if (!conv1(box[l][1], first.sub(0, cb), b2, hs[l], ws[l], 1) || !head(box[l][2], b2, 1, hs[l], ws[l], a0, strides[l])) return false;
+                if (tail_k) { if (!conv_head(cls[l][1], cls[l][2], first.sub(cb, cc), 2, hs[l], ws[l], a0, strides[l])) return false; }
+                else if (!conv1(cls[l][1], first.sub(cb, cc), k2, hs[l], ws[l], 1) || !head(cls[l][2], k2, 2, hs[l], ws[l], a0, strides[l])) return false;
             } else {
                 View bo = buf(m, rm4), ko = buf(m, d.nc);
                 if (!bo.base || !ko.base) return false;
@@ -429,6 +451,10 @@
             return rva_yolo_head3_box32_f16(c, s.hb, s.hldb, s.hk, s.hldc, output, boxes, n, s.hh, s.hw, p->nc, p->A, s.hs, st);
     }
     switch (s.kind) {
+    case K_CONV_HEAD:
+        if (!output) return RVA_ERR_ARG;
+        return rva_conv3x3_head_f16_sel(c, s.in, s.ldi, s.w, s.b, s.w2, s.b2, n, p->B, s.H, s.W, s.Cin, s.Cout, s.mode, p->nc, output,
+                                        p->box32 && s.mode == 1 ? (float *)((char *)output + p->box_off) : nullptr, p->A, s.a0, s.stride_px, variant, st);
     case K_CONV: return rva_conv2d_nhwc_f16_sel(c, s.in, s.ldi, s.w, s.b, s.out, s.ldo, s.res, s.ldr, n, p->B, s.H, s.W, s.Cin, s.Cout, s.k, s.stride, s.act, variant,
                                                 0, -1, st);
     case K_UPCAT: return rva_conv1x1_upcat_f16(c, s.in, s.ldi, s.c_in, s.in2, s.ldi2, s.c_in2, s.w, s.b, s.out, s.ldo, n, s.H, s.W, s.Cout, s.act, variant, st);
@@ -452,6 +478,7 @@
 bool variant_fits(const Step &s, int variant)
 {
     if (s.kind == K_CONV) return variant >= 0;
+    if (s.kind == K_CONV_HEAD) return variant >= 0 && rva_conv_variant_tail(variant, s.Cout);
     if (s.kind == K_CONV_F32) return variant >= 0 && variant <= rva_conv_f32_num_variants();
     return variant == 0 || rva_conv_variant_is_gather64(variant);
 }
@@ -672,7 +699,7 @@
     if (!p || index < 0 || index >= (int)p->tunables.size()) return RVA_ERR_ARG;
     const Step &s = p->steps[p->tunables[index].step];
     if (!variant_fits(s, variant)) return RVA_ERR_ARG;
-    if (s.kind == K_HEAD && !output) return RVA_ERR_ARG;
+    if ((s.kind == K_HEAD || s.kind == K_CONV_HEAD) && !output) return RVA_ERR_ARG;
     return launch_step(p, s, variant, nullptr, output, p->B, stream, true);
 }
 
diff --git a/realtime_video_analytics_32streams_amd/detector.py b/realtime_video_analytics_32streams_amd/detector.py
--- a/realtime_video_analytics_32streams_amd/detector.py
+++ b/realtime_video_analytics_32streams_amd/detector.py
@@ -178,11 +178,16 @@
             plan = self._plans[key] = FusedYoloV8(self.net, shape[0], shape[1:], device=self.device, ctx=self.ctx,
                                                   autotune=first is None, tune_overlap=getattr(self, "tune_overlap", 1),
                                                   precision="fp32" if self.engine == "fused-f32" else "fp16", box_rows=self.box_rows,
-                                                  static_rows=rows if self.engine == "fused" else None)
+                                                  static_rows=rows if self.engine == "fused" else None, head_tails=self._head_tails())
             if first is not None:
                 plan.copy_tuning(first)
         plan.n = batch
         return plan
+
+    def _head_tails(self) -> int:
+        import os
+        from .engine import HEAD_TAILS_PRODUCTION
+        return HEAD_TAILS_PRODUCTION if self.engine == "fused" and os.environ.get("RVA_PLAN_NO_HEAD_TAILS") != "1" else 0
 
     def rows_pending(self, batch: int) -> bool:
         return not self._rows_told.get(self._buf_key(batch), True)
diff --git a/realtime_video_analytics_32streams_amd/engine.py b/realtime_video_analytics_32streams_amd/engine.py
--- a/realtime_video_analytics_32streams_amd/engine.py
+++ b/realtime_video_analytics_32streams_amd/engine.py
@@ -14,6 +14,8 @@
 
 
 _LIB_DIGEST: Optional[str] = None
+
+HEAD_TAILS_PRODUCTION = N.RVA_PLAN_TAIL_ALL
 
 
 def _lib_digest() -> str:
@@ -64,7 +66,7 @@
 class FusedYoloV8:
     def __init__(self, net: YoloV8, batch: int, hw: Tuple[int, int] = (640, 640), device: Optional[torch.device] = None,
                  ctx: Optional[N.Context] = None, autotune: bool = True, tune_overlap: int = 1, precision: str = "fp16",
-                 box_rows: str = "fp16", static_rows: Optional[Tuple[int, int]] = None):
+                 box_rows: str = "fp16", static_rows: Optional[Tuple[int, int]] = None, head_tails: int = 0):
         import os
         if precision not in ("fp16", "fp32"):
             raise ValueError(f"precision must be 'fp16' or 'fp32', not {precision!r}")
@@ -72,6 +74,9 @@
             raise ValueError(f"box_rows must be 'fp16' or 'fp32', not {box_rows!r}")
         if box_rows == "fp32" and precision == "fp32":
             raise ValueError("box_rows='fp32' belongs to the fp16 plan: the output of precision='fp32' is fp32 already")
+        if head_tails & ~N.RVA_PLAN_TAIL_ALL:
+            raise ValueError(f"head_tails must be a mask of RVA_PLAN_TAIL_BOX / RVA_PLAN_TAIL_CLS bits, not {head_tails:#x}")
+        self.head_tails = 0 if precision == "fp32" else int(head_tails)
         self.box_rows = box_rows
         self.precision = precision
         self.f32 = precision == "fp32"
@@ -105,7 +110,7 @@
         d.flags = (N.RVA_PLAN_NO_STEM2 if os.environ.get("RVA_NO_STEM2", "0") == "1" else 0) | \
                   (N.RVA_PLAN_NO_CIN_PAD if os.environ.get("RVA_NO_CIN_PAD", "0") == "1" else 0) | \
                   (0 if self._use_pair32() else N.RVA_PLAN_NO_PAIR32) | \
-                  (N.RVA_PLAN_F32 if self.f32 else 0) | (N.RVA_PLAN_BOX_F32 if box_rows == "fp32" else 0)
+                  (N.RVA_PLAN_F32 if self.f32 else 0) | (N.RVA_PLAN_BOX_F32 if box_rows == "fp32" else 0) | self.head_tails
         h = C.c_void_p()
         with torch.cuda.device(self.dev):
             self.ctx.check(self.L.rva_yolov8_plan_create(self.ctx.handle, C.byref(d), arr, C.byref(h)), "rva_yolov8_plan_create")
@@ -204,6 +209,8 @@
         h.update(repr(int(os.environ.get("RVA_TUNE_LAYER_OVERLAP", getattr(self, "tune_overlap", 1)))).encode())
         if getattr(self, "f32", False):
             h.update(b"precision fp32")
+        if getattr(self, "head_tails", 0):
+            h.update(f"head tails {self.head_tails:#x}".encode())
         return h.hexdigest()[:24]
 
     def _load_tuning(self) -> bool:
@@ -325,7 +332,7 @@
         n_over = int(os.environ.get("RVA_TUNE_OVERLAP", "3"))
         if n_over >= 2:
             twins = [FusedYoloV8(self._net, self.B, (self.H, self.W), device=self.dev, ctx=self.ctx, autotune=False, precision=self.precision,
-                                 box_rows=self.box_rows, static_rows=self.static_rows)
+                                 box_rows=self.box_rows, static_rows=self.static_rows, head_tails=self.head_tails)
                      for _ in range(n_over - 1)]
             from .ops import chain_streams
             streams = chain_streams(self.dev, n_over)
```

After: 24230, median of 3. No clear change (+0.6%).
